# Hysocs/Aozora_SDXL_Training

Hardware: AMD Instinct MI355X
Metric: SDXL UNet train iters/sec (1024px, gbs=32) (higher is better)
Workload: dtype bf16; 1 GPU; SDXL-base UNet (2.567B params), epsilon pred, 1024x1024 (latent 4x128x128), ctx 77x2048, local batch 4 x grad-accum 8 x 1 GPU = global batch 32, Raven AdamW (bf16 m/v resident in HBM -- 10.3 GB of 288; the reference parks them in pinned host memory to fit 24 GB cards: other_configs.cfg2_state_on_host of --full --, sharded 1/N per rank), clip 1.0, eager 2-stream issue (dgrad chain || wgrad branch); global_batch=32, parallelism=dp1

## Files before the change

aozora_sdxl_training_amd/_lib.py:

```python
from __future__ import annotations

import ctypes
import os
import re
from typing import Callable, Dict, List, NamedTuple, Tuple

_HERE = os.path.dirname(os.path.abspath(__file__))
_ROOT = os.path.dirname(_HERE)
HEADER = os.path.join(_ROOT, "include", "aozora_hip.h")
LIB_PATH = os.path.join(_HERE, "libaozora_hip.so")

_CTYPES = {
    "int": ctypes.c_int, "long": ctypes.c_long, "float": ctypes.c_float,
    "void*": ctypes.c_void_p, "const void*": ctypes.c_void_p,
    "void**": ctypes.POINTER(ctypes.c_void_p), "int*": ctypes.POINTER(ctypes.c_int),
    "float*": ctypes.POINTER(ctypes.c_float), "const char*": ctypes.c_char_p, "long*": ctypes.POINTER(ctypes.c_long),
}


def parse_header(path: str = HEADER) -> Dict[str, Tuple[str, List[Tuple[str, str]]]]:
    src = open(path).read()
    src = re.sub(r"/\*.*?\*/", "", src, flags=re.S)
    protos = {}
    for m in re.finditer(r"\b(int|long)\s+(az_\w+)\s*\(([^)]*)\)\s*;", src):
        ret, name, args = m.group(1), m.group(2), m.group(3).strip()
        alist = []
        if args and args != "void":
            for a in args.split(","):
                a = " ".join(a.split())
                mm = re.match(r"(.*?)(\w+)$", a)
                ty = mm.group(1).strip().replace(" *", "*")
                alist.append((ty, mm.group(2)))
        protos[name] = (ret, alist)
    return protos


class AozoraError(RuntimeError):
    pass


class Call(NamedTuple):
    name: str
    args: tuple


class Record(NamedTuple):
    event: object
    stream: object


class Wait(NamedTuple):
    stream: object
    event: object


class Live(NamedTuple):
    fn: Callable
    args: tuple


class _Lib:
    def __init__(self):
        if not os.path.exists(LIB_PATH):
            raise AozoraError(
                f"{LIB_PATH} is missing: build it with `python -c 'import __graft_entry__ as g; g.build()'` "
                "(hipcc --offload-arch=gfx950). There is no CPU fallback for the HIP path.")
        self.cdll = ctypes.CDLL(LIB_PATH)
        self.protos = parse_header()
        self._fn = {}
        for name, (ret, args) in self.protos.items():
            fn = getattr(self.cdll, name)
            fn.restype = _CTYPES[ret]
            fn.argtypes = [_CTYPES[t] for t, _ in args]
            self._fn[name] = fn
        self.recorder = None

    def call(self, name: str, *args):
        fn = self._fn[name]
        rc = fn(*args)
        if rc != 0:
            raise AozoraError(f"{name} failed with code {rc}" + (" (argument error)" if rc <= -1000 else " (HIP error)"))
        if self.recorder is not None:
            self.recorder.append(Call(name, args))
        return rc

    def raw(self, name: str):
        return getattr(self.cdll, name)


def set_option(name: str, value: int):
    L = lib()
    rc = L._fn["az_set_option"](name.encode(), int(value))
    if rc != 0:
        raise AozoraError(f"az_set_option({name!r}) failed with code {rc}")


def get_option(name: str) -> int:
    v = ctypes.c_int()
    rc = lib()._fn["az_get_option"](name.encode(), ctypes.byref(v))
    if rc != 0:
        raise AozoraError(f"az_get_option({name!r}) failed with code {rc}")
    return v.value


class ForkEvent:
    __slots__ = ("cuda_event",)

    def __init__(self):
        h = ctypes.c_void_p()
        rc = lib()._fn["az_event_create_fork"](ctypes.byref(h))
        if rc != 0:
            raise AozoraError(f"az_event_create_fork failed with code {rc}")
        self.cuda_event = h.value

    def record(self, stream):
        rc = lib()._fn["az_event_record"](self.cuda_event, stream.cuda_stream)
        if rc != 0:
            raise AozoraError(f"az_event_record failed with code {rc}")

    def wait(self, stream):
        rc = lib()._fn["az_stream_wait_event"](stream.cuda_stream, self.cuda_event)
        if rc != 0:
            raise AozoraError(f"az_stream_wait_event failed with code {rc}")

    wait_on = wait

    def destroy(self):
        if self.cuda_event:
            lib()._fn["az_event_destroy"](self.cuda_event)
            self.cuda_event = None


_lib = None


def lib() -> _Lib:
    global _lib
    if _lib is None:
        _lib = _Lib()
    return _lib
```

aozora_sdxl_training_amd/csrc/az_common.h:

```cpp
#pragma once
#include <hip/hip_runtime.h>
#include <hip/hip_ext.h>
#include <stdint.h>
#include <tuple>
#include <utility>

typedef uint16_t bf16_t;
typedef __attribute__((ext_vector_type(8))) short bf16x8;
typedef __attribute__((ext_vector_type(4))) short bf16x4;
typedef __attribute__((ext_vector_type(4))) float f32x4;
typedef __attribute__((ext_vector_type(16))) float f32x16;
typedef __attribute__((ext_vector_type(4))) unsigned int u32x4;

#define AZ_OK 0
#define AZ_ERR_ARG(k) (-1000 - (k))

#define AZ_CHECK_LAUNCH()                          \
  do {                                             \
    hipError_t _e = hipGetLastError();             \
    if (_e != hipSuccess) return -(int)_e;         \
  } while (0)

hipEvent_t az_stop_event_of_this_thread();
template <typename... P, size_t... I>
// ... 25 lines not shown

__device__ __forceinline__ uint32_t pack2bf(float lo, float hi) {
  return (uint32_t)f2bf(lo) | ((uint32_t)f2bf(hi) << 16);
}

__device__ __forceinline__ float silu_f(float x) { return x * __builtin_amdgcn_rcpf(1.0f + __expf(-x)); }
__device__ __forceinline__ float dsilu_f(float x) {
  float s = __builtin_amdgcn_rcpf(1.0f + __expf(-x));
  return s * (1.0f + x * (1.0f - s));
}

__device__ __forceinline__ void gelu_pair(float g, float& gelu, float& dgelu) {
  const float x = fabsf(g) * 0.70710678118654752f;
  const float t = __builtin_amdgcn_rcpf(fmaf(0.3275911f, x, 1.0f));
  const float e = __expf(-x * x);
  const float poly = t * fmaf(t, fmaf(t, fmaf(t, fmaf(t, 1.061405429f, -1.453152027f), 1.421413741f), -0.284496736f), 0.254829592f);
  const float hc = 0.5f * poly * e;
  const float phi = g >= 0.f ? 1.0f - hc : hc;
  gelu = g * phi;
  dgelu = fmaf(g * 0.3989422804014327f, e, phi);
}
__device__ __forceinline__ float gelu_erf(float g) { float a, b; gelu_pair(g, a, b); return a; }
__device__ __forceinline__ float dgelu_erf(float g) { float a, b; gelu_pair(g, a, b); return b; }

__device__ __forceinline__ void divmod(long i, int d, long& q, int& r) {
  if ((unsigned long)i <= 0xFFFFFFFFul) {
    const unsigned qi = (unsigned)i / (unsigned)d;
    q = (long)qi; r = (int)((unsigned)i - qi * (unsigned)d);
  } else {
    q = i / d; r = (int)(i - q * d);
  }
}

__device__ __forceinline__ float wave_sum(float v) {
#pragma unroll
  for (int o = 32; o > 0; o >>= 1) v += __shfl_xor(v, o, 64);
  return v;
}
__device__ __forceinline__ float wave_max(float v) {
#pragma unroll
  for (int o = 32; o > 0; o >>= 1) v = fmaxf(v, __shfl_xor(v, o, 64));
  return v;
}

__device__ __forceinline__ float block_sum(float v, float* sh) {
  v = wave_sum(v);
  int w = threadIdx.x >> 6, nw = (blockDim.x + 63) >> 6;
  __syncthreads();
  if ((threadIdx.x & 63) == 0) sh[w] = v;
  __syncthreads();
  float r = 0.f;
  for (int i = 0; i < nw; ++i) r += sh[i];
  return r;
}

__device__ __forceinline__ bf16x4 lds_read_tr16_b64(uint32_t lds_byte_addr) {
  bf16x4 v;
  asm volatile("ds_read_b64_tr_b16 %0, %1" : "=v"(v) : "v"(lds_byte_addr) : "memory");
  return v;
}

enum AzOption {
  AZ_OPT_TILE_POLICY = 0,
  AZ_OPT_BIG_FILL,
  AZ_OPT_SPLIT_SLOTS,
  AZ_OPT_NOSPLIT_TILES,
  AZ_OPT_LDS_EXCLUSIVE,
  AZ_OPT_NT_SPLIT_BIG,
  AZ_OPT_NT_SPLIT_MINK,
  AZ_OPT_ATTN_SPLIT_TARGET,
  AZ_OPT_LN_RPB,
  AZ_OPT_INKERNEL_FINISH,
  AZ_OPT_NT_SPLIT2_MINK,
  AZ_OPT_GEMM_ABLATE,
  AZ_OPT_GEMM8,
  AZ_OPT_NT_SPLIT_FWD,
  AZ_OPT_ATTN_PIPE,
  AZ_OPT_XCD_SPLIT,
  AZ_OPT_ATTN_XCD,
  AZ_OPT_NORM_STAT_BF16,
  AZ_OPT_GN_RPT,
  AZ_OPT_GN_RPT_BWD,
  AZ_OPT_GN_RPT_APPLY,
  AZ_OPT_COUNT
};
int az_opt(int id);
```

aozora_sdxl_training_amd/csrc/az_gemm.hip:

```cpp
#include "az_common.h"
#include "aozora_hip.h"
#include <cstdlib>
#include <type_traits>

namespace {

constexpr int BK = 64;
constexpr int PITCH_K = BK * 2;
constexpr int PITCH_X = 128 * 2;

enum { A_ROW = 0, A_COL = 1, A_CONV = 2, A_CONVT = 3 };
enum { B_NT = 0, B_NN = 1, B_CONVDG = 2, B_CONVWG = 3 };

struct Geom {
  int Hin, Win, Cin;
  int Hout, Wout, Cout;
  int stride, pad, ks;
  int cpad;
  int ups;
};

struct Params {
  const bf16_t* A; const bf16_t* B;
  long lda, ldb;
// ... 1039 lines not shown
  if (g_force_bm == 256 && g_force_nw == 8) {
    p.bm = 256; p.bn = 256; p.nwaves = 0;
    return;
  }
  if (g_force_bm) {
    const bool kb32 = ((g_force_nw >> 5) & 1) && b_kmajor, deep = (g_force_nw >> 4) & 1;
    p.bm = g_force_bm; p.bn = g_force_bn; p.nwaves = g_force_nw & 15;
    p.kb = kb32 ? 32 : 64; p.stages = kb32 ? (deep ? 5 : 4) : (deep ? 3 : 2);
    if ((g_force_nw >> 6) & 1) { p.kb = 64; p.stages = 4; }
    if (p.bn == 160 && !b_kmajor) { p.bn = 128; p.nwaves = 8; p.stages = 2; }
    if (((g_force_nw >> 5) & 1) && !b_kmajor && p.bm == 256) { p.nwaves = 0; p.stages = 2; }
    return;
  }
  const int policy = az_opt(AZ_OPT_TILE_POLICY);
  const bool exclusive = az_opt(AZ_OPT_LDS_EXCLUSIVE) != 0;
  p.bm = 128; p.bn = 128; p.nwaves = 8;
  if (wgrad) return;
  const long t256 = (long)((p.M + 255) / 256) * ((p.N + 255) / 256);
  const long waves = (t256 + 255) / 256;
  const bool big = t256 * 10 >= waves * 256 * az_opt(AZ_OPT_BIG_FILL);
  if (b_kmajor && (p.N % 160) == 0 && (p.N <= 640 || !big)) {
    p.bn = 160; p.nwaves = 8;
    const long t160 = (long)((p.M + 127) / 128) * (p.N / 160);
    if ((policy >= 5 || exclusive) && t160 <= 256 && p.N > 640) p.stages = 3;
    return;
  }
  if (big) { p.bm = 256; p.bn = 256; p.nwaves = 0; }
}

int choose_split(Params& p, int want_split, long ws_bytes, bool wgrad = false, bool b_kmajor = false, bool big_split = false) {
  if (big_split) { p.bm = 256; p.bn = 256; p.nwaves = 0; p.stages = 2; p.kb = 64; }
  else choose_tile(p, wgrad, b_kmajor);
  p.tiles_m = (p.M + p.bm - 1) / p.bm;
  p.tiles_n = (p.N + p.bn - 1) / p.bn;
  const int ktiles = (p.K + BK - 1) / BK;
  int s = 1;
  if (want_split != 1 && p.ws) {
    const int tiles = p.tiles_m * p.tiles_n;
    if (want_split > 1) {
      s = want_split;
    } else {
      const int slots = az_opt(AZ_OPT_SPLIT_SLOTS);
      double best = -1.0;
      const int nosplit = az_opt(AZ_OPT_NOSPLIT_TILES);
      for (int c = 1; c <= (tiles >= nosplit ? 1 : 24); ++c) {
        if (c > 1 && ktiles / c < 8) break;
        const long blocks = (long)tiles * c;
        const double fill = (double)blocks / (double)(((blocks + slots - 1) / slots) * slots);
        const double score = fill / (1.0 + 0.08 * (c - 1));
        if (score > best + 1e-9) { best = score; s = c; }
      }
    }
    if (s > ktiles) s = ktiles;
    if (s > 64) s = 64;
    while (s > 1 && (long)s * p.M * p.N * 4 > ws_bytes) --s;
    if (s < 1) s = 1;
  }
  p.ktiles_per_split = (ktiles + s - 1) / s;
  p.ksplit = (ktiles + p.ktiles_per_split - 1) / p.ktiles_per_split;
  if (p.ksplit < 1) p.ksplit = 1;
  p.xsplit = (wgrad && az_opt(AZ_OPT_XCD_SPLIT) != 0 && p.ksplit > 1) ? 1 : 0;
  p.wgrad_c = wgrad ? 1 : 0;
  return AZ_OK;
}

void apply_gemm8(Params& p, int want_bn = 0) {
  p.use8 = 0;
  const bool forced = (g_force_bm == 256 && g_force_nw == 8);
  if (!forced && (g_force_bm || !az_opt(AZ_OPT_GEMM8))) return;
  if (p.bm != 256 || p.bn != 256 || (p.K % BK) || p.rowbias || !vec_epi_ok(p)) return;
  int bn = 256;
  if (forced) {
    bn = (g_force_bn == 320 && (p.N % 320) == 0) ? 320 : 256;
  } else if (want_bn) {
    bn = want_bn;
  } else if ((p.N % 320) == 0 && p.ksplit == 1) {
    auto fill = [&](int w) { const long tl = (long)((p.M + 255) / 256) * ((p.N + w - 1) / w); return (double)tl / (double)(((tl + 255) / 256) * 256); };
    if (fill(320) > fill(256) + 1e-9) bn = 320;
  }
  p.use8 = 1; p.bn = bn;
  p.tiles_m = (p.M + 255) / 256; p.tiles_n = (p.N + bn - 1) / bn;
}

}

extern "C" {

int az_gemm_set_exclusive(int on) { return az_set_option("LDS_EXCLUSIVE", on ? 1 : 0); }

int az_gemm_set_tile(int bm, int bn) { return az_gemm_set_tile_ex(bm, bn, 0); }

int az_gemm_set_tile_ex(int bm, int bn, int waves) {
  const bool std_tile = (bm == 128 && bn == 128 && (waves == 0 || waves == 8)) ||
                        (bm == 256 && bn == 256 && (waves == 0 || waves == 32 || waves == 8)) ||
                        (bm == 256 && bn == 320 && waves == 8);
  const bool n160 = (bm == 128 && bn == 160 && (waves == 0 || waves == 8 || waves == 24 ||
                                                waves == 40 || waves == 56 || waves == 72));
  if (!((bm == 0 && bn == 0) || std_tile || n160)) return AZ_ERR_ARG(9);
  g_force_bm = bm; g_force_bn = bn; g_force_nw = waves;
  return AZ_OK;
}

constexpr long TICKET_BYTES = 16384;
static void carve_tickets(Params& p, void* workspace, long& workspace_bytes) {
  p.tickets = nullptr;
  if (!workspace || workspace_bytes < TICKET_BYTES + 65536 || ((uintptr_t)workspace & 15) || (workspace_bytes & 15)) return;
  if (!az_opt(AZ_OPT_INKERNEL_FINISH)) return;
  workspace_bytes -= TICKET_BYTES;
  p.tickets = (unsigned*)((char*)workspace + workspace_bytes);
}

static int carve_colsum(Params& p, void* workspace, long& workspace_bytes, int nseg, int rps) {
  const long need = 64L * nseg * p.M * 4;
  if (!workspace || workspace_bytes < need + 4096 || ((uintptr_t)workspace & 15)) return AZ_ERR_ARG(20);
  if (nseg > 1 && (rps % BK)) return AZ_ERR_ARG(21);
  workspace_bytes = ((workspace_bytes - need) / 16) * 16;
  p.cs_ws = (float*)((char*)workspace + workspace_bytes);
  p.cs_nseg = nseg; p.cs_rps = rps;
  return AZ_OK;
}

static int gemm_impl(int transA, int transB, int M, int N, int K, const void* A, long lda, const void* B, long ldb,
                 void* C, long ldc, const void* bias, const void* rowbias, int rows_per_seg, long ld_rowbias,
                 const void* residual, long ldr, int accumulate, int split_k, void* workspace, long workspace_bytes,
                 void* bias_grad, int n_real, void* stream) {
  if (M <= 0 || N <= 0 || K <= 0) return AZ_ERR_ARG(1);
  if ((K & 7) && !transA && !transB) return AZ_ERR_ARG(2);
  if ((lda & 7) || (ldb & 7)) return AZ_ERR_ARG(3);
  if (((uintptr_t)A & 15) || ((uintptr_t)B & 15)) return AZ_ERR_ARG(4);
  if (rowbias && rows_per_seg <= 0) return AZ_ERR_ARG(5);
  Params p{};
  p.A = (const bf16_t*)A; p.B = (const bf16_t*)B; p.lda = lda; p.ldb = ldb; p.M = M; p.N = N; p.K = K;
  p.C = (bf16_t*)C; p.ldc = ldc; p.ws = (float*)workspace; p.bias = (const bf16_t*)bias;
  p.rowbias = (const bf16_t*)rowbias; p.rows_per_seg = rows_per_seg; p.ld_rb = ld_rowbias;
  p.R = (const bf16_t*)residual; p.ldr = ldr; p.accumulate = accumulate;
  carve_tickets(p, workspace, workspace_bytes);
  if (bias_grad) {
    if (!(transA && !transB) || n_real > M) return AZ_ERR_ARG(22);
    int rc0 = carve_colsum(p, workspace, workspace_bytes, 1, K);
    if (rc0) return rc0;
    p.cs_bias = (bf16_t*)bias_grad; p.cs_n_real = n_real; p.cs_seg_out = nullptr;
  }
  bool big_split = false; int split_bn = 256;
  {
    const int sb = az_opt(AZ_OPT_LDS_EXCLUSIVE) ? az_opt(AZ_OPT_NT_SPLIT_FWD) : az_opt(AZ_OPT_NT_SPLIT_BIG);
    if (sb > 1 && !transA && transB && !g_force_bm && !rowbias && workspace && (K % BK) == 0 && K >= az_opt(AZ_OPT_NT_SPLIT_MINK) &&
        (split_k == 0 || split_k == 1) && (!residual || (((ldr & 7) == 0) && (((uintptr_t)residual & 15) == 0))) &&
        ((N & 7) == 0) && ((ldc & 7) == 0) && (((uintptr_t)C & 15) == 0) && (((uintptr_t)workspace & 15) == 0)) {
      const int kt = K / BK;
      double best = 0.0; int bs = 0;
      for (int bn = 256; bn <= 320; bn += 64) {
        if (bn == 320 && ((N % 320) || !az_opt(AZ_OPT_GEMM8))) continue;
        const long tl = (long)((M + 255) / 256) * ((N + bn - 1) / bn);
        if (tl > 128) continue;
        for (int sp = 2; sp <= sb; ++sp) {
          if (kt / sp < 8 || tl * sp > 256 || (long)sp * M * N * 4 > workspace_bytes) break;
          const double score = (double)(tl * sp) / 256.0 - 0.02 * (sp - 1);
          if (score > best + 1e-9) { best = score; bs = sp; split_bn = bn; }
        }
      }
      if (bs > 1 && best >= 0.7) { big_split = true; split_k = bs; }
    }
  }
  if (!big_split && !transA && transB && !g_force_bm && !rowbias && !residual && workspace && (K % BK) == 0 && (split_k == 0 || split_k == 1) &&
      !az_opt(AZ_OPT_LDS_EXCLUSIVE) && az_opt(AZ_OPT_TILE_POLICY) < 5) {
    const int mink = az_opt(AZ_OPT_NT_SPLIT2_MINK);
    const long t256 = (long)((M + 255) / 256) * ((N + 255) / 256);
    const long t160 = (long)((M + 127) / 128) * (N / 160);
    const bool big = t256 * 10 >= ((t256 + 255) / 256) * 256 * az_opt(AZ_OPT_BIG_FILL);
    if (mink > 0 && K >= mink && (N % 160) == 0 && N > 640 && !big && t160 <= 256 && 2L * M * N * 4 <= workspace_bytes - 65536) split_k = 2;
  }
  choose_split(p, split_k, workspace_bytes, transA != 0, !transA && transB, big_split);
  if (p.ksplit > 1 && (rowbias || (residual && !vec_epi_ok(p)))) return AZ_ERR_ARG(6);
  if (!transA && transB) apply_gemm8(p, big_split ? split_bn : 0);
  if ((long)p.tiles_m * p.tiles_n > TICKET_BYTES / 4 || (long)p.ksplit * p.M * p.N * 4 >= 0x7FFFFFF0L || p.use8 || (p.R && p.ksplit > 1)) p.tickets = nullptr;
  hipStream_t st = (hipStream_t)stream;
  if (p.tickets) AZ_HIP(hipMemsetAsync(p.tickets, 0, (size_t)p.tiles_m * p.tiles_n * 4, st));
  int rc;
  if (!transA && transB) rc = launch<A_ROW, B_NT>(p, st);
  else if (!transA && !transB) rc = launch<A_ROW, B_NN>(p, st);
  else if (transA && !transB) rc = launch<A_COL, B_NN>(p, st);
  else return AZ_ERR_ARG(7);
  if (rc) return rc;
  return finish_product(p, st, nullptr, bias_grad, n_real);
}

int az_gemm_bf16(int transA, int transB, int M, int N, int K, const void* A, long lda, const void* B, long ldb,
                 void* C, long ldc, const void* bias, const void* rowbias, int rows_per_seg, long ld_rowbias,
                 const void* residual, long ldr, int accumulate, int split_k, void* workspace, long workspace_bytes,
                 void* stream) {
  return gemm_impl(transA, transB, M, N, K, A, lda, B, ldb, C, ldc, bias, rowbias, rows_per_seg, ld_rowbias, residual, ldr,
                   accumulate, split_k, workspace, workspace_bytes, nullptr, 0, stream);
}

int az_gemm_geglu_fwd_bf16(int M, int H, int K, const void* X, long lda, const void* W, long ldb, const void* bias, void* proj, long ldp,
                           void* out, long ldo, void* stream) {
  if (M <= 0 || H <= 0 || K <= 0 || (K & 7) || (H & 7)) return AZ_ERR_ARG(72);
  if ((lda & 7) || (ldb & 7) || (ldp & 7) || (ldo & 7)) return AZ_ERR_ARG(73);
  if (((uintptr_t)X & 15) || ((uintptr_t)W & 15) || ((uintptr_t)proj & 15) || ((uintptr_t)out & 15) || !proj || !out) return AZ_ERR_ARG(74);
  Params p{};
  p.A = (const bf16_t*)X; p.B = (const bf16_t*)W; p.lda = lda; p.ldb = ldb; p.M = M; p.N = 2 * H; p.K = K;
  p.C = (bf16_t*)proj; p.ldc = ldp; p.bias = (const bf16_t*)bias; p.gg_H = H; p.gg_y = (bf16_t*)out; p.gg_ldy = ldo;
  choose_split(p, 1, 0, false, true);
  const bool big = (p.bm == 256 && p.bn == 256);
  p.stages = 2; p.kb = 64;
  if (!big) { p.bm = 128; p.bn = 128; }
  p.nwaves = big ? 0 : 8;
  p.tiles_m = (M + p.bm - 1) / p.bm; p.tiles_n = (H + p.bn / 2 - 1) / (p.bn / 2);
  p.use8 = (big && (K % BK) == 0 && vec_epi_ok(p) && (az_opt(AZ_OPT_GEMM8) || (g_force_bm == 256 && g_force_nw == 8)) &&
            (!g_force_bm || g_force_nw == 8)) ? 1 : 0;
  return launch<A_ROW, B_NT>(p, (hipStream_t)stream);
}

int az_gemm_nt_grouped_bf16(int M, int K, const void* A, long lda, const void* groups_dev, int ngroups, long total_tiles_n, void* stream) {
  if (M <= 0 || K <= 0 || (K & 7) || (lda & 7) || ((uintptr_t)A & 15) || !groups_dev || ngroups <= 0 || total_tiles_n <= 0 ||
      ((uintptr_t)groups_dev & 7)) return AZ_ERR_ARG(70);
  Params p{};
  p.A = (const bf16_t*)A; p.lda = lda; p.M = M; p.K = K; p.N = 0;
  p.groups = (const GemmGroup*)groups_dev; p.ngroups = ngroups;
  p.bm = 128; p.bn = 160; p.nwaves = 8; p.kb = 64;
  p.stages = az_opt(AZ_OPT_LDS_EXCLUSIVE) ? 3 : 2;
  p.tiles_m = (M + 127) / 128;
  if ((long)p.tiles_m * total_tiles_n > 0x7FFFFFF0L) return AZ_ERR_ARG(71);
  p.tiles_n = (int)total_tiles_n;
  p.ksplit = 1; p.ktiles_per_split = (K + BK - 1) / BK;
  if ((long)M * lda * 2 >= 0x7FFFFFF0L) return AZ_ERR_ARG(8);
  p.lda2 = (int)(lda * 2);
  p.k_full = (K % BK) == 0;
  p.vec_epi = 1;
  hipStream_t st = (hipStream_t)stream;
  if (p.stages == 3) return launch_tile<A_ROW, B_NT, 128, 160, 4, 2, 3, 64, 1>(p, st);
  return launch_tile<A_ROW, B_NT, 128, 160, 4, 2, 2, 64, 1>(p, st);
}

int az_gemm_tn_grouped_bf16(const void* groups_dev, int ngroups, long total_tiles, void* stream) {
  if (!groups_dev || ngroups <= 0 || total_tiles <= 0 || total_tiles > 0x7FFFFFF0L || ((uintptr_t)groups_dev & 7)) return AZ_ERR_ARG(75);
  Params p{};
  p.tgroups = (const TnGroup*)groups_dev; p.ngroups = ngroups;
  p.bm = 128; p.bn = 128; p.nwaves = 8; p.kb = 64; p.stages = 2;
  p.tiles_m = (int)total_tiles; p.tiles_n = 1;
  p.ksplit = 1; p.accumulate = 1;
  return launch_tile<A_COL, B_NN, 128, 128, 4, 2, 2, 64, 3>(p, (hipStream_t)stream);
}

int az_gemm_wgrad_bias_bf16(int M, int N, int K, const void* dY, long lddy, const void* X, long ldx, void* dW, long lddw,
                            int accumulate, int split_k, void* workspace, long workspace_bytes, void* bias_grad, int n_real,
                            void* stream) {
  if (!bias_grad) return AZ_ERR_ARG(22);
  return gemm_impl(1, 0, M, N, K, dY, lddy, X, ldx, dW, lddw, nullptr, nullptr, 0, 0, nullptr, 0, accumulate, split_k, workspace,
                   workspace_bytes, bias_grad, n_real, stream);
}

static int conv_impl(int mode, int batch, int Hin, int Win, int Cin, int Hout, int Wout, int Cout, int ksize, int stride,
                   int pad, int cpad, const void* X, long ldx, const void* W, const void* dY, long lddy, void* out,
                   long ldo, const void* bias, const void* rowbias, long ld_rowbias, const void* residual, long ldr,
                   int accumulate, int split_k, void* workspace, long workspace_bytes, void* bias_grad, void* seg_grad,
                   void* stream) {
  const int ups = (mode >> 4) & 1;
  mode &= 15;
  if (ups && ((mode != 0 && mode != 2) || ksize != 3 || stride != 1 || (Hin & 1) || (Win & 1))) return AZ_ERR_ARG(23);
  if (ksize != 1 && ksize != 3) return AZ_ERR_ARG(10);
  if (stride != 1 && stride != 2) return AZ_ERR_ARG(11);
  if ((Cin & 7)) return AZ_ERR_ARG(12);
  Params p{};
  p.g = Geom{Hin, Win, Cin, Hout, Wout, Cout, stride, pad, ksize, cpad > 0 ? cpad : Cout, ups};
  const int taps = ksize * ksize;
  p.bias = (const bf16_t*)bias; p.accumulate = accumulate; p.ws = (float*)workspace;
  p.rowbias = (const bf16_t*)rowbias; p.ld_rb = ld_rowbias; p.R = (const bf16_t*)residual; p.ldr = ldr;
  hipStream_t st = (hipStream_t)stream;
  int rc;
  if (mode == 0) {
    p.A = (const bf16_t*)X; p.lda = ldx; p.B = (const bf16_t*)W; p.ldb = (long)taps * Cin;
    p.M = batch * Hout * Wout; p.N = Cout; p.K = taps * Cin; p.C = (bf16_t*)out; p.ldc = ldo;
    p.rows_per_seg = Hout * Wout;
    p.tap_uniform = (Cin % BK) == 0;
// ... 70 lines not shown
```

aozora_sdxl_training_amd/csrc/az_norm.hip:

```cpp
#include "az_common.h"
#include "aozora_hip.h"

namespace {

constexpr int GN_MAX_THREADS = 256;

struct GnGeom {
  int B, HW, C, G, cpg, cchunks, py, rows_per_chunk, nchunk;
  int stat_bf16;
};

__device__ __forceinline__ float stat_round(float v, int on) { return on ? bf2f(f2bf(v)) : v; }

constexpr int GN_RPT_MIN = 4;
__host__ GnGeom gn_geom(int B, int HW, int C, int G, int pass = -1) {
  GnGeom g;
  g.B = B; g.HW = HW; g.C = C; g.G = G; g.cpg = C / G; g.cchunks = C / 8;
  g.py = GN_MAX_THREADS / g.cchunks; if (g.py < 1) g.py = 1;
  int want = (HW + 1023) / 1024;
  int rpt = pass < 0 ? GN_RPT_MIN : az_opt(pass == 2 ? AZ_OPT_GN_RPT_APPLY : pass ? AZ_OPT_GN_RPT_BWD : AZ_OPT_GN_RPT);
  if (rpt < GN_RPT_MIN) rpt = GN_RPT_MIN; if (rpt > 64) rpt = 64;
  if (want < rpt * g.py) want = rpt * g.py;
  g.rows_per_chunk = ((want + g.py - 1) / g.py) * g.py;
  g.nchunk = (HW + g.rows_per_chunk - 1) / g.rows_per_chunk;
// ... 287 lines not shown
      ub[i] = *reinterpret_cast<const uint4*>(beta + cc * 8);
      unpack8(ux, v[i]);
#pragma unroll
      for (int e = 0; e < 8; ++e) s += v[i][e];
    }
  }
  const float invC = 1.0f / (float)C;
  const float mean = wave_sum(s) * invC;
  float q = 0.f;
#pragma unroll
  for (int i = 0; i < LN_MAXCH; ++i) {
    int cc = lane + 64 * i;
    if (cc < cch) {
#pragma unroll
      for (int e = 0; e < 8; ++e) { float d = v[i][e] - mean; q += d * d; }
    }
  }
  const float rstd = rsqrtf(fmaf(wave_sum(q), invC, eps));
  if (lane == 0) { stats[row * 2] = stat_round(mean, stat_bf16); stats[row * 2 + 1] = stat_round(rstd, stat_bf16); }
#pragma unroll
  for (int i = 0; i < LN_MAXCH; ++i) {
    int cc = lane + 64 * i;
    if (cc < cch) {
      float g8[8], b8[8], o[8];
      unpack8(ug[i], g8);
      unpack8(ub[i], b8);
#pragma unroll
      for (int e = 0; e < 8; ++e) o[e] = (v[i][e] - mean) * rstd * g8[e] + b8[e];
      *reinterpret_cast<uint4*>(y + (long)row * ldy + cc * 8) = pack8(o);
    }
  }
}

template <int NCH>
__global__ __launch_bounds__(256) void ln_bwd_dx_kernel(int M, int C, const bf16_t* __restrict__ x, long ldx, const bf16_t* __restrict__ gamma,
                                 const float* __restrict__ stats, const bf16_t* __restrict__ dy, long lddy,
                                 bf16_t* dx, long lddx, const bf16_t* dadd, long ldadd) {
  const bool accumulate = dadd != nullptr;
  const int lane = threadIdx.x & 63;
  const int row = blockIdx.x * (blockDim.x >> 6) + (threadIdx.x >> 6);
  if (row >= M) return;
  const int cch = C >> 3;
  const float mean = stats[row * 2], rstd = stats[row * 2 + 1];
  float xh[NCH][8], dg[NCH][8];
  uint4 prev[NCH];
  float c1 = 0.f, c2 = 0.f;
#pragma unroll
  for (int i = 0; i < NCH; ++i) {
    const int cc = lane + 64 * i;
    if (cc < cch) {
      const uint4 ux = *reinterpret_cast<const uint4*>(x + (long)row * ldx + cc * 8);
      const uint4 ud = *reinterpret_cast<const uint4*>(dy + (long)row * lddy + cc * 8);
      const uint4 ug = *reinterpret_cast<const uint4*>(gamma + cc * 8);
      if (accumulate) prev[i] = *reinterpret_cast<const uint4*>(dadd + (long)row * ldadd + cc * 8);
      float f[8], d[8], g8[8];
      unpack8(ux, f); unpack8(ud, d); unpack8(ug, g8);
#pragma unroll
      for (int e = 0; e < 8; ++e) {
        xh[i][e] = (f[e] - mean) * rstd;
        dg[i][e] = d[e] * g8[e];
        c1 += dg[i][e]; c2 += dg[i][e] * xh[i][e];
      }
    }
  }
  const float invC = 1.0f / (float)C;
  c1 = wave_sum(c1) * invC; c2 = wave_sum(c2) * invC;
#pragma unroll
  for (int i = 0; i < NCH; ++i) {
    const int cc = lane + 64 * i;
    if (cc < cch) {
      float o[8];
      bf16_t* op = dx + (long)row * lddx + cc * 8;
      if (accumulate) unpack8(prev[i], o);
#pragma unroll
      for (int e = 0; e < 8; ++e) {
        float vv = rstd * (dg[i][e] - c1 - xh[i][e] * c2);
        o[e] = accumulate ? o[e] + vv : vv;
      }
      *reinterpret_cast<uint4*>(op) = pack8(o);
    }
  }
}

template <int NCH>
__global__ __launch_bounds__(256) void ln_bwd_fused_kernel(int M, int C, int rows_per_block, const bf16_t* __restrict__ x, long ldx,
                                 const bf16_t* __restrict__ gamma, const float* __restrict__ stats, const bf16_t* __restrict__ dy,
                                 long lddy, bf16_t* dx, long lddx, const bf16_t* dadd, long ldadd, float* __restrict__ partial) {
  const bool accumulate = dadd != nullptr;
  extern __shared__ float sh[];
  const int lane = threadIdx.x & 63, w = threadIdx.x >> 6;
  const int cch = C >> 3;
  const int r0 = blockIdx.x * rows_per_block;
  int r1 = r0 + rows_per_block; if (r1 > M) r1 = M;
  float pg[NCH][8], pb[NCH][8];
  uint4 ug[NCH];
#pragma unroll
  for (int i = 0; i < NCH; ++i) {
    const int cc = lane + 64 * i;
    ug[i] = cc < cch ? *reinterpret_cast<const uint4*>(gamma + cc * 8) : make_uint4(0, 0, 0, 0);
#pragma unroll
    for (int e = 0; e < 8; ++e) { pg[i][e] = 0.f; pb[i][e] = 0.f; }
  }
  const float invC = 1.0f / (float)C;
  uint4 nx[NCH], nd[NCH], np[NCH];
  float nmean = 0.f, nrstd = 0.f;
  auto fetch = [&](int row) {
    nmean = stats[row * 2]; nrstd = stats[row * 2 + 1];
#pragma unroll
    for (int i = 0; i < NCH; ++i) {
      const int cc = lane + 64 * i;
      if (cc < cch) {
        nx[i] = *reinterpret_cast<const uint4*>(x + (long)row * ldx + cc * 8);
        nd[i] = *reinterpret_cast<const uint4*>(dy + (long)row * lddy + cc * 8);
        if (accumulate) np[i] = *reinterpret_cast<const uint4*>(dadd + (long)row * ldadd + cc * 8);
      }
    }
  };
  if (r0 + w < r1) fetch(r0 + w);
  for (int row = r0 + w; row < r1; row += 4) {
    const float mean = nmean, rstd = nrstd;
    uint4 cx[NCH], cd[NCH], prev[NCH];
#pragma unroll
    for (int i = 0; i < NCH; ++i) { cx[i] = nx[i]; cd[i] = nd[i]; if (accumulate) prev[i] = np[i]; }
    if (row + 4 < r1) fetch(row + 4);
    float xh[NCH][8], dg[NCH][8];
    float c1 = 0.f, c2 = 0.f;
#pragma unroll
    for (int i = 0; i < NCH; ++i) {
      const int cc = lane + 64 * i;
      if (cc < cch) {
        float f[8], d[8], g8[8];
        unpack8(cx[i], f); unpack8(cd[i], d); unpack8(ug[i], g8);
#pragma unroll
        for (int e = 0; e < 8; ++e) {
          xh[i][e] = (f[e] - mean) * rstd;
          pb[i][e] += d[e]; pg[i][e] += d[e] * xh[i][e];
          dg[i][e] = d[e] * g8[e];
          c1 += dg[i][e]; c2 += dg[i][e] * xh[i][e];
        }
      }
    }
    c1 = wave_sum(c1) * invC; c2 = wave_sum(c2) * invC;
#pragma unroll
    for (int i = 0; i < NCH; ++i) {
      const int cc = lane + 64 * i;
      if (cc < cch) {
        float o[8];
        if (accumulate) unpack8(prev[i], o);
#pragma unroll
        for (int e = 0; e < 8; ++e) {
          float vv = rstd * (dg[i][e] - c1 - xh[i][e] * c2);
          o[e] = accumulate ? o[e] + vv : vv;
        }
        *reinterpret_cast<uint4*>(dx + (long)row * lddx + cc * 8) = pack8(o);
      }
    }
  }
  float* out = partial + (long)blockIdx.x * C * 2;
#pragma unroll
  for (int i = 0; i < NCH; ++i) {
    if (i) __syncthreads();
    float* d = sh + ((long)w * 64 + lane) * 16;
#pragma unroll
    for (int e = 0; e < 8; e += 2)
      *reinterpret_cast<float4*>(d + e * 2) = make_float4(pg[i][e], pb[i][e], pg[i][e + 1], pb[i][e + 1]);
    __syncthreads();
    const int l2 = threadIdx.x >> 2, q = threadIdx.x & 3;
    const int cc = l2 + 64 * i;
    if (cc < cch) {
      float4 a = *reinterpret_cast<const float4*>(sh + (long)l2 * 16 + q * 4);
#pragma unroll
      for (int y = 1; y < 4; ++y) {
        const float4 v = *reinterpret_cast<const float4*>(sh + ((long)y * 64 + l2) * 16 + q * 4);
        a.x += v.x; a.y += v.y; a.z += v.z; a.w += v.w;
      }
      *reinterpret_cast<float4*>(out + ((long)cc * 8 + q * 2) * 2) = a;
    }
  }
}

__global__ void ln_bwd_param_kernel(int M, int C, int rows_per_block, const bf16_t* __restrict__ x, long ldx,
                                    const float* __restrict__ stats, const bf16_t* __restrict__ dy, long lddy,
                                    float* __restrict__ partial) {
  extern __shared__ float sh[];
  const int cc = blockIdx.y * blockDim.x + threadIdx.x;
  const int cch = C >> 3;
  const int r0 = blockIdx.x * rows_per_block;
  int r1 = r0 + rows_per_block; if (r1 > M) r1 = M;
  float dg[8], db[8];
#pragma unroll
  for (int e = 0; e < 8; ++e) { dg[e] = 0.f; db[e] = 0.f; }
  if (cc < cch) {
#pragma unroll 4
    for (int r = r0 + threadIdx.y; r < r1; r += blockDim.y) {
      const float mean = stats[r * 2], rstd = stats[r * 2 + 1];
      float f[8], d[8];
      unpack8(*reinterpret_cast<const uint4*>(x + (long)r * ldx + cc * 8), f);
      unpack8(*reinterpret_cast<const uint4*>(dy + (long)r * lddy + cc * 8), d);
#pragma unroll
      for (int e = 0; e < 8; ++e) { db[e] += d[e]; dg[e] += d[e] * (f[e] - mean) * rstd; }
    }
  }
  const int w8 = blockDim.x * 8;
#pragma unroll
  for (int e = 0; e < 8; ++e) {
    sh[((threadIdx.y * w8) + threadIdx.x * 8 + e) * 2] = dg[e];
    sh[((threadIdx.y * w8) + threadIdx.x * 8 + e) * 2 + 1] = db[e];
  }
  __syncthreads();
  const int tid = threadIdx.y * blockDim.x + threadIdx.x, nth = blockDim.x * blockDim.y;
  for (int lc = tid; lc < w8; lc += nth) {
    const int c = blockIdx.y * w8 + lc;
    if (c >= C) continue;
    float a = 0.f, bsum = 0.f;
    for (int y = 0; y < (int)blockDim.y; ++y) { a += sh[(y * w8 + lc) * 2]; bsum += sh[(y * w8 + lc) * 2 + 1]; }
    partial[((long)blockIdx.x * C + c) * 2] = a;
    partial[((long)blockIdx.x * C + c) * 2 + 1] = bsum;
  }
}

__device__ __forceinline__ void colpair_finalize_block(int blk, int nparts, int C, const float* __restrict__ partial, bf16_t* dgamma, bf16_t* dbeta,
                                                       float4 (*sh)[16]) {
  const int lc = threadIdx.x & 15, sl = threadIdx.x >> 4;
  const int c = blk * 32 + lc * 2;
  float4 a = make_float4(0.f, 0.f, 0.f, 0.f);
  if (c < C) {
    const float* base = partial + (long)c * 2;
    int k = sl;
    for (; k + 7 * 16 < nparts; k += 8 * 16) {
      float4 v[8];
#pragma unroll
      for (int u = 0; u < 8; ++u) v[u] = *reinterpret_cast<const float4*>(base + (long)(k + u * 16) * C * 2);
#pragma unroll
      for (int u = 0; u < 8; ++u) { a.x += v[u].x; a.y += v[u].y; a.z += v[u].z; a.w += v[u].w; }
    }
    for (; k < nparts; k += 16) {
      const float4 v = *reinterpret_cast<const float4*>(base + (long)k * C * 2);
      a.x += v.x; a.y += v.y; a.z += v.z; a.w += v.w;
    }
  }
  sh[sl][lc] = a;
  __syncthreads();
  if (sl == 0 && c < C) {
    a = make_float4(0.f, 0.f, 0.f, 0.f);
#pragma unroll
    for (int i = 0; i < 16; ++i) { const float4 v = sh[i][lc]; a.x += v.x; a.y += v.y; a.z += v.z; a.w += v.w; }
    if (dgamma) { dgamma[c] = f2bf(bf2f(dgamma[c]) + a.x); dgamma[c + 1] = f2bf(bf2f(dgamma[c + 1]) + a.z); }
    if (dbeta) { dbeta[c] = f2bf(bf2f(dbeta[c]) + a.y); dbeta[c + 1] = f2bf(bf2f(dbeta[c + 1]) + a.w); }
  }
}
// ... 57 lines not shown
                       (const bf16_t*)beta, (const float*)stats, (bf16_t*)y, ldy);
  AZ_CHECK_LAUNCH();
  return AZ_OK;
}

int az_groupnorm_bwd_ex(int batch, int HW, int C, int G, int fuse_silu, const void* x, long ldx, const void* gamma,
                        const void* beta, const void* stats, const void* dy, long lddy, void* dx, long lddx,
                        const void* dx_add, long ld_add, void* dgamma, void* dbeta, void* partial, void* stream) {
  int rc = gn_check(batch, HW, C, G, ldx); if (rc) return rc;
  if ((lddy & 7) || (lddx & 7) || (dx_add && (ld_add & 7)) || ((uintptr_t)gamma & 15) || ((uintptr_t)beta & 15) || ((uintptr_t)stats & 7)) return AZ_ERR_ARG(25);
  GnGeom g = gn_geom(batch, HW, C, G, 1);
  hipStream_t st = (hipStream_t)stream;
  dim3 blk(g.cchunks, g.py), grid(g.nchunk, batch);
  size_t shb = (size_t)g.py * C * 2 * sizeof(float);
  if (shb > 64 * 1024) return AZ_ERR_ARG(24);
  float* part = (float*)partial;
  float* chan = part + (long)batch * g.nchunk * C * 2;
  float* gsum = chan + (long)batch * C * 2;
  if (fuse_silu)
    az_launch(gn_bwd_partial_kernel<true>, grid, blk, shb, st, g, (const bf16_t*)x, ldx, (const bf16_t*)gamma,
                       (const bf16_t*)beta, (const float*)stats, (const bf16_t*)dy, lddy, part);
  else
    az_launch(gn_bwd_partial_kernel<false>, grid, blk, shb, st, g, (const bf16_t*)x, ldx, (const bf16_t*)gamma,
                       (const bf16_t*)beta, (const float*)stats, (const bf16_t*)dy, lddy, part);
  AZ_CHECK_LAUNCH();
  az_launch(gn_bwd_finalize_kernel, dim3(G, batch), dim3(64, 16), 0, st, g, (const bf16_t*)gamma, (const float*)part, chan, gsum);
  AZ_CHECK_LAUNCH();
  const bool params = dgamma || dbeta;
  if (params && !dx) {
    az_launch(gn_bwd_param_kernel, dim3((C + 255) / 256), dim3(256), 0, st, g, (const float*)chan, (bf16_t*)dgamma, (bf16_t*)dbeta);
    AZ_CHECK_LAUNCH();
  }
  const float* chan_for_apply = params ? chan : nullptr;
  if (dx) {
    g = gn_geom(batch, HW, C, G, 2);
    blk = dim3(g.cchunks, g.py); grid = dim3(g.nchunk, batch);
    if (fuse_silu)
      az_launch(gn_bwd_apply_kernel<true>, grid, blk, 0, st, g, (const bf16_t*)x, ldx, (const bf16_t*)gamma,
                         (const bf16_t*)beta, (const float*)stats, (const float*)gsum, (const bf16_t*)dy, lddy,
                         (bf16_t*)dx, lddx, (const bf16_t*)dx_add, ld_add, chan_for_apply, (bf16_t*)dgamma, (bf16_t*)dbeta);
    else
      az_launch(gn_bwd_apply_kernel<false>, grid, blk, 0, st, g, (const bf16_t*)x, ldx, (const bf16_t*)gamma,
                         (const bf16_t*)beta, (const float*)stats, (const float*)gsum, (const bf16_t*)dy, lddy,
                         (bf16_t*)dx, lddx, (const bf16_t*)dx_add, ld_add, chan_for_apply, (bf16_t*)dgamma, (bf16_t*)dbeta);
    AZ_CHECK_LAUNCH();
  }
  return AZ_OK;
}

int az_groupnorm_bwd(int batch, int HW, int C, int G, int fuse_silu, const void* x, long ldx, const void* gamma,
                     const void* beta, const void* stats, const void* dy, long lddy, void* dx, long lddx,
                     int accumulate_dx, void* dgamma, void* dbeta, void* partial, void* stream) {
  return az_groupnorm_bwd_ex(batch, HW, C, G, fuse_silu, x, ldx, gamma, beta, stats, dy, lddy, dx, lddx, accumulate_dx ? dx : nullptr, lddx,
                             dgamma, dbeta, partial, stream);
}

long az_ln_scratch_floats(int M, int C) { (void)M; return (long)LN_FUSED_MAX_BLOCKS * C * 2; }

int az_layernorm_fwd(int M, int C, float eps, const void* x, long ldx, const void* gamma, const void* beta, void* y,
                     long ldy, void* stats, void* stream) {
  if (M <= 0 || (C & 7) || C > 64 * 8 * LN_MAXCH || (ldx & 7) || (ldy & 7)) return AZ_ERR_ARG(30);
  az_launch(ln_fwd_kernel, dim3((M + 3) / 4), dim3(256), 0, (hipStream_t)stream, M, C, eps, (const bf16_t*)x, ldx,
                     (const bf16_t*)gamma, (const bf16_t*)beta, (bf16_t*)y, ldy, (float*)stats, (int)(az_opt(AZ_OPT_NORM_STAT_BF16) != 0));
  AZ_CHECK_LAUNCH();
  return AZ_OK;
}

static int ln_fused_rpb(int M);
int az_layernorm_bwd_ex(int M, int C, const void* x, long ldx, const void* gamma, const void* stats, const void* dy,
                        long lddy, void* dx, long lddx, const void* dx_add, long ld_add, void* dgamma, void* dbeta, void* partial,
                        void* stream) {
  if (M <= 0 || (C & 7) || C > 64 * 8 * LN_MAXCH || (ldx & 7) || (lddy & 7) || (dx && (lddx & 7)) || (dx_add && (ld_add & 7))) return AZ_ERR_ARG(31);
  hipStream_t st = (hipStream_t)stream;
  const int cch = C / 8;
  const int nch = (cch + 63) / 64;
  dim3 g1((M + 3) / 4), b1(256);
#define LN_DX(N) az_launch(ln_bwd_dx_kernel<N>, g1, b1, 0, st, M, C, (const bf16_t*)x, ldx, (const bf16_t*)gamma, \
                                    (const float*)stats, (const bf16_t*)dy, lddy, (bf16_t*)dx, lddx, (const bf16_t*)dx_add, ld_add)
  if (dx && (dgamma || dbeta)) {
    const int nblk = (M + ln_fused_rpb(M) - 1) / ln_fused_rpb(M);
    const int rpb = ((M + nblk - 1) / nblk + 3) / 4 * 4;
    const size_t shb = (size_t)4 * 64 * 16 * sizeof(float);
#define LN_FU(N) az_launch(ln_bwd_fused_kernel<N>, dim3(nblk), b1, shb, st, M, C, rpb, (const bf16_t*)x, ldx, (const bf16_t*)gamma, \
                                    (const float*)stats, (const bf16_t*)dy, lddy, (bf16_t*)dx, lddx, (const bf16_t*)dx_add, ld_add, (float*)partial)
    if (nch == 1) LN_FU(1); else if (nch == 2) LN_FU(2); else if (nch == 3) LN_FU(3); else LN_FU(4);
#undef LN_FU
    AZ_CHECK_LAUNCH();
    az_launch(colpair_finalize_kernel, dim3((C + 31) / 32), dim3(256), 0, st, nblk, C, (const float*)partial,
                       (bf16_t*)dgamma, (bf16_t*)dbeta);
    AZ_CHECK_LAUNCH();
    return AZ_OK;
  }
  if (dx) {
    if (nch == 1) LN_DX(1); else if (nch == 2) LN_DX(2); else if (nch == 3) LN_DX(3); else LN_DX(4);
    AZ_CHECK_LAUNCH();
  }
#undef LN_DX
  if (dgamma || dbeta) {
    int bx = cch < 128 ? cch : 128; int by = 256 / bx; if (by < 1) by = 1; if (by > 16) by = 16;
    int colblocks = (cch + bx - 1) / bx;
    int rpb = (M + LN_BWD_BLOCKS - 1) / LN_BWD_BLOCKS; if (rpb < by) rpb = by;
    int nblk = (M + rpb - 1) / rpb;
    size_t shb = (size_t)by * bx * 8 * 2 * sizeof(float);
    az_launch(ln_bwd_param_kernel, dim3(nblk, colblocks), dim3(bx, by), shb, st, M, C, rpb, (const bf16_t*)x, ldx,
                       (const float*)stats, (const bf16_t*)dy, lddy, (float*)partial);
    AZ_CHECK_LAUNCH();
    az_launch(colpair_finalize_kernel, dim3((C + 31) / 32), dim3(256), 0, st, nblk, C, (const float*)partial,
                       (bf16_t*)dgamma, (bf16_t*)dbeta);
    AZ_CHECK_LAUNCH();
  }
  return AZ_OK;
}

static int ln_fused_rpb(int M) {
  const int rpb_env = az_opt(AZ_OPT_LN_RPB);
  int rpb = rpb_env < 4 ? 4 : (rpb_env + 3) / 4 * 4;
  while ((M + rpb - 1) / rpb > LN_FUSED_MAX_BLOCKS) rpb += 4;
  return rpb;
}

int az_ln_partial_blocks(int M) { return M > 0 ? (M + ln_fused_rpb(M) - 1) / ln_fused_rpb(M) : 0; }

int az_layernorm_bwd_partial(int M, int C, const void* x, long ldx, const void* gamma, const void* stats, const void* dy,
                             long lddy, void* dx, long lddx, const void* dx_add, long ld_add, void* partial, int nblk, void* stream) {
  if (M <= 0 || (C & 7) || C > 64 * 8 * LN_MAXCH || (ldx & 7) || (lddy & 7) || !dx || (lddx & 7) || (dx_add && (ld_add & 7)) || !partial) return AZ_ERR_ARG(32);
  if (nblk <= 0 || nblk > LN_FUSED_MAX_BLOCKS) return AZ_ERR_ARG(34);
  const int rpb = ((M + nblk - 1) / nblk + 3) / 4 * 4;
  if ((M + rpb - 1) / rpb != nblk) return AZ_ERR_ARG(34);
  hipStream_t st = (hipStream_t)stream;
  const int nch = (C / 8 + 63) / 64;
  const size_t shb = (size_t)4 * 64 * 16 * sizeof(float);
#define LN_FU(N) az_launch(ln_bwd_fused_kernel<N>, dim3(nblk), dim3(256), shb, st, M, C, rpb, (const bf16_t*)x, ldx, (const bf16_t*)gamma, \
                                    (const float*)stats, (const bf16_t*)dy, lddy, (bf16_t*)dx, lddx, (const bf16_t*)dx_add, ld_add, (float*)partial)
  if (nch == 1) LN_FU(1); else if (nch == 2) LN_FU(2); else if (nch == 3) LN_FU(3); else LN_FU(4);
#undef LN_FU
  AZ_CHECK_LAUNCH();
  return AZ_OK;
}

int az_ln_param_finish_multi(const void* jobs_dev, int njobs, long nblocks, void* stream) {
  if (!jobs_dev || njobs <= 0 || nblocks <= 0 || nblocks > 0x7FFFFFF0L || ((uintptr_t)jobs_dev & 7)) return AZ_ERR_ARG(33);
  az_launch(colpair_finalize_multi_kernel, dim3((unsigned)nblocks), dim3(256), 0, (hipStream_t)stream, (const LnFinishJob*)jobs_dev, njobs);
  AZ_CHECK_LAUNCH();
  return AZ_OK;
}

int az_layernorm_bwd(int M, int C, const void* x, long ldx, const void* gamma, const void* stats, const void* dy,
                     long lddy, void* dx, long lddx, int accumulate_dx, void* dgamma, void* dbeta, void* partial,
                     void* stream) {
  return az_layernorm_bwd_ex(M, C, x, ldx, gamma, stats, dy, lddy, dx, lddx, accumulate_dx ? dx : nullptr, lddx, dgamma, dbeta, partial, stream);
}

}
```

aozora_sdxl_training_amd/csrc/az_runtime.hip:

```cpp
#include "az_common.h"
#include "aozora_hip.h"
#include <string.h>
#include <stdlib.h>
#include <atomic>
#include <mutex>

namespace {
struct OptDef { const char* name; int def; };
const OptDef OPT_DEFS[AZ_OPT_COUNT] = {
  {"TILE_POLICY", 4}, {"BIG_FILL", 5}, {"SPLIT_SLOTS", 384}, {"NOSPLIT_TILES", 256}, {"LDS_EXCLUSIVE", 0}, {"NT_SPLIT_BIG", 3},
  {"NT_SPLIT_MINK", 5120}, {"ATTN_SPLIT_TARGET", 384}, {"LN_RPB", 32}, {"INKERNEL_FINISH", 0}, {"NT_SPLIT2_MINK", 0}, {"GEMM_ABLATE", 0}, {"GEMM8", 1}, {"NT_SPLIT_FWD", 0}, {"ATTN_PIPE", 15}, {"XCD_SPLIT", 1}, {"ATTN_XCD", 15}, {"NORM_STAT_BF16", 1}, {"GN_RPT", 4}, {"GN_RPT_BWD", 32}, {"GN_RPT_APPLY", 32},
};
std::atomic<int> g_opt[AZ_OPT_COUNT];
std::once_flag g_opt_once;
void opt_init() {
  for (int i = 0; i < AZ_OPT_COUNT; ++i) {
    char key[64];
    snprintf(key, sizeof key, "AZ_%s", OPT_DEFS[i].name);
    const char* e = getenv(key);
    g_opt[i].store(e ? atoi(e) : OPT_DEFS[i].def, std::memory_order_relaxed);
  }
}

__global__ void spin_kernel(long ticks) {
  const long t0 = (long)wall_clock64();
  while ((long)wall_clock64() - t0 < ticks) __builtin_amdgcn_s_sleep(32);
}
}

struct AzContext { int device; std::atomic<int> refs; std::atomic<int> opt[AZ_OPT_COUNT]; };
static void ctx_release(AzContext* c) {
  if (c && c->refs.fetch_sub(1, std::memory_order_acq_rel) == 1) delete c;
}
struct AzCurrent {
  AzContext* c = nullptr;
  ~AzCurrent() { ctx_release(c); }
  operator AzContext*() const { return c; }
  AzContext* operator->() const { return c; }
  void set(AzContext* n) {
    if (n == c) return;
    if (n) n->refs.fetch_add(1, std::memory_order_relaxed);
    AzContext* old = c; c = n;
    ctx_release(old);
  }
};
static thread_local AzCurrent t_ctx;

int az_opt(int id) {
  std::call_once(g_opt_once, opt_init);
  AzContext* c = t_ctx.c;
  return c ? c->opt[id].load(std::memory_order_relaxed) : g_opt[id].load(std::memory_order_relaxed);
}

struct AzStopEvent { hipEvent_t ev = nullptr; long launches = 0; };
static AzStopEvent& az_stop_event_slot() {
  static thread_local AzStopEvent s;
  return s;
}
hipEvent_t az_stop_event_of_this_thread() {
  AzStopEvent& s = az_stop_event_slot();
  if (s.ev) ++s.launches;
  return s.ev;
}

extern "C" {

int az_version(void) { return 101; }

int az_set_option(const char* name, int value) {
  std::call_once(g_opt_once, opt_init);
  if (!name) return AZ_ERR_ARG(91);
  std::atomic<int>* tab = t_ctx.c ? t_ctx.c->opt : g_opt;
  for (int i = 0; i < AZ_OPT_COUNT; ++i)
    if (!strcmp(name, OPT_DEFS[i].name)) { tab[i].store(value, std::memory_order_relaxed); return AZ_OK; }
  return AZ_ERR_ARG(92);
}

int az_get_option(const char* name, int* value) {
  std::call_once(g_opt_once, opt_init);
  if (!name || !value) return AZ_ERR_ARG(91);
  std::atomic<int>* tab = t_ctx.c ? t_ctx.c->opt : g_opt;
  for (int i = 0; i < AZ_OPT_COUNT; ++i)
    if (!strcmp(name, OPT_DEFS[i].name)) { *value = tab[i].load(std::memory_order_relaxed); return AZ_OK; }
  return AZ_ERR_ARG(92);
}

int az_init(int device, void** handle) {
  std::call_once(g_opt_once, opt_init);
  if (!handle || device < 0) return AZ_ERR_ARG(93);
  AzContext* c = new AzContext;
  c->device = device;
  c->refs.store(1, std::memory_order_relaxed);
  for (int i = 0; i < AZ_OPT_COUNT; ++i) c->opt[i].store(g_opt[i].load(std::memory_order_relaxed), std::memory_order_relaxed);
  *handle = c;
// ... 111 lines not shown
```

aozora_sdxl_training_amd/csrc/az_tape_dispatch.inc:

```
static const char* const AZ_TAPE_FN_NAMES[] = {
  "az_adamw8bit_step",
  "az_adamw_flat",
  "az_adamw_flat_ex",
  "az_add_rows",
  "az_attn_bwd",
  "az_attn_fwd",
  "az_clip_coef",
  "az_colsum",
  "az_colsum_grad",
  "az_conv2d_bf16",
  "az_conv2d_wgrad_bias_bf16",
  "az_destroy",
  "az_event_destroy",
  "az_event_record",
  "az_event_sync",
  "az_f32_to_bf16",
  "az_geglu_bwd",
  "az_geglu_fwd",
  "az_gemm_bf16",
  "az_gemm_geglu_fwd_bf16",
  "az_gemm_nt_grouped_bf16",
  "az_gemm_set_exclusive",
  "az_gemm_set_tile",
  "az_gemm_set_tile_ex",
  "az_gemm_tn_grouped_bf16",
  "az_gemm_wgrad_bias_bf16",
  "az_graph_begin",
  "az_graph_destroy",
  "az_graph_launch",
  "az_groupnorm_bwd",
  "az_groupnorm_bwd_ex",
  "az_groupnorm_fwd",
  "az_host_free",
  "az_layernorm_bwd",
  "az_layernorm_bwd_ex",
  "az_layernorm_bwd_partial",
  "az_layernorm_fwd",
  "az_ln_param_finish_multi",
  "az_ln_partial_blocks",
  "az_make_current",
  "az_memcpy_async",
  "az_memset_async",
  "az_mse_loss_fwd_bwd",
  "az_nchw_to_nhwc_pad",
  "az_nhwc_to_nchw",
  "az_noise_target",
  "az_raven_step",
  "az_raven_step_ex",
  "az_reduce_segs_to_bf16",
  "az_scale_bf16",
  "az_scale_f32",
  "az_set_launch_stop_event",
  "az_silu_bwd",
  "az_silu_fwd",
  "az_spin",
  "az_stage_inputs",
  "az_stream_sync",
  "az_stream_wait_event",
  "az_sumsq",
  "az_sumsq_bf16",
  "az_timestep_embed",
  "az_titan_offload",
  "az_transpose_bf16",
  "az_transpose_bf16_batched",
  "az_transpose_multi_bf16",
  "az_upsample2x_bwd",
  "az_upsample2x_fwd",
  "az_version",
};
static const int AZ_TAPE_FN_NARGS[] = {7, 9, 10, 9, 35, 19, 6, 8, 10, 29, 22, 1, 1, 2, 1, 4, 9, 7, 22, 13, 8, 1, 2, 3, 4, 16, 1, 1, 2, 19, 20, 15, 1, 15, 16, 15, 11, 4, 1, 1, 5, 4, 14, 8, 8, 12, 13, 14, 6, 4, 4, 1, 6, 4, 2, 8, 1, 2, 7, 6, 6, 6, 7, 10, 4, 7, 7, 0};
static int az_tape_dispatch(int fn, const long* w) {
  switch (fn) {
    case 0: return az_adamw8bit_step((int)w[0], (const void*)w[1], (long)w[2], (const void*)w[3], (const void*)w[4], (const void*)w[5], (void*)w[6]);
    case 1: return az_adamw_flat((long)w[0], (void*)w[1], (const void*)w[2], (void*)w[3], (void*)w[4], (int)w[5], (const void*)w[6], (const void*)w[7], (void*)w[8]);
    case 2: return az_adamw_flat_ex((long)w[0], (void*)w[1], (const void*)w[2], (int)w[3], (void*)w[4], (void*)w[5], (int)w[6], (const void*)w[7], (const void*)w[8], (void*)w[9]);
    case 3: return az_add_rows((long)w[0], (int)w[1], (const void*)w[2], (long)w[3], (const void*)w[4], (long)w[5], (void*)w[6], (long)w[7], (void*)w[8]);
    case 4: return az_attn_bwd((int)w[0], (int)w[1], (int)w[2], (int)w[3], word_float(w[4]), (const void*)w[5], (long)w[6], (long)w[7], (const void*)w[8], (long)w[9], (long)w[10], (const void*)w[11], (long)w[12], (long)w[13], (const void*)w[14], (long)w[15], (long)w[16], (const void*)w[17], (long)w[18], (long)w[19], (const void*)w[20], (void*)w[21], (void*)w[22], (long)w[23], (long)w[24], (void*)w[25], (long)w[26], (long)w[27], (void*)w[28], (long)w[29], (long)w[30], (void*)w[31], (long)w[32], (int)w[33], (void*)w[34]);
    case 5: return az_attn_fwd((int)w[0], (int)w[1], (int)w[2], (int)w[3], word_float(w[4]), (const void*)w[5], (long)w[6], (long)w[7], (const void*)w[8], (long)w[9], (long)w[10], (const void*)w[11], (long)w[12], (long)w[13], (void*)w[14], (long)w[15], (long)w[16], (void*)w[17], (void*)w[18]);
    case 6: return az_clip_coef((const void*)w[0], word_float(w[1]), word_float(w[2]), (void*)w[3], (void*)w[4], (void*)w[5]);
    case 7: return az_colsum((long)w[0], (int)w[1], (int)w[2], (const void*)w[3], (long)w[4], (void*)w[5], (void*)w[6], (void*)w[7]);
    case 8: return az_colsum_grad((long)w[0], (int)w[1], (int)w[2], (const void*)w[3], (long)w[4], (void*)w[5], (void*)w[6], (int)w[7], (void*)w[8], (void*)w[9]);
    case 9: return az_conv2d_bf16((int)w[0], (int)w[1], (int)w[2], (int)w[3], (int)w[4], (int)w[5], (int)w[6], (int)w[7], (int)w[8], (int)w[9], (int)w[10], (int)w[11], (const void*)w[12], (long)w[13], (const void*)w[14], (const void*)w[15], (long)w[16], (void*)w[17], (long)w[18], (const void*)w[19], (const void*)w[20], (long)w[21], (const void*)w[22], (long)w[23], (int)w[24], (int)w[25], (void*)w[26], (long)w[27], (void*)w[28]);
    case 10: return az_conv2d_wgrad_bias_bf16((int)w[0], (int)w[1], (int)w[2], (int)w[3], (int)w[4], (int)w[5], (int)w[6], (int)w[7], (int)w[8], (int)w[9], (const void*)w[10], (long)w[11], (const void*)w[12], (long)w[13], (void*)w[14], (int)w[15], (int)w[16], (void*)w[17], (long)w[18], (void*)w[19], (void*)w[20], (void*)w[21]);
    case 11: return az_destroy((void*)w[0]);
    case 12: return az_event_destroy((void*)w[0]);
    case 13: return az_event_record((void*)w[0], (void*)w[1]);
    case 14: return az_event_sync((void*)w[0]);
    case 15: return az_f32_to_bf16((long)w[0], (const void*)w[1], (void*)w[2], (void*)w[3]);
    case 16: return az_geglu_bwd((int)w[0], (int)w[1], (const void*)w[2], (long)w[3], (const void*)w[4], (long)w[5], (void*)w[6], (long)w[7], (void*)w[8]);
    case 17: return az_geglu_fwd((int)w[0], (int)w[1], (const void*)w[2], (long)w[3], (void*)w[4], (long)w[5], (void*)w[6]);
    case 18: return az_gemm_bf16((int)w[0], (int)w[1], (int)w[2], (int)w[3], (int)w[4], (const void*)w[5], (long)w[6], (const void*)w[7], (long)w[8], (void*)w[9], (long)w[10], (const void*)w[11], (const void*)w[12], (int)w[13], (long)w[14], (const void*)w[15], (long)w[16], (int)w[17], (int)w[18], (void*)w[19], (long)w[20], (void*)w[21]);
    case 19: return az_gemm_geglu_fwd_bf16((int)w[0], (int)w[1], (int)w[2], (const void*)w[3], (long)w[4], (const void*)w[5], (long)w[6], (const void*)w[7], (void*)w[8], (long)w[9], (void*)w[10], (long)w[11], (void*)w[12]);
    case 20: return az_gemm_nt_grouped_bf16((int)w[0], (int)w[1], (const void*)w[2], (long)w[3], (const void*)w[4], (int)w[5], (long)w[6], (void*)w[7]);
    case 21: return az_gemm_set_exclusive((int)w[0]);
    case 22: return az_gemm_set_tile((int)w[0], (int)w[1]);
    case 23: return az_gemm_set_tile_ex((int)w[0], (int)w[1], (int)w[2]);
    case 24: return az_gemm_tn_grouped_bf16((const void*)w[0], (int)w[1], (long)w[2], (void*)w[3]);
    case 25: return az_gemm_wgrad_bias_bf16((int)w[0], (int)w[1], (int)w[2], (const void*)w[3], (long)w[4], (const void*)w[5], (long)w[6], (void*)w[7], (long)w[8], (int)w[9], (int)w[10], (void*)w[11], (long)w[12], (void*)w[13], (int)w[14], (void*)w[15]);
    case 26: return az_graph_begin((void*)w[0]);
    case 27: return az_graph_destroy((void*)w[0]);
    case 28: return az_graph_launch((void*)w[0], (void*)w[1]);
    case 29: return az_groupnorm_bwd((int)w[0], (int)w[1], (int)w[2], (int)w[3], (int)w[4], (const void*)w[5], (long)w[6], (const void*)w[7], (const void*)w[8], (const void*)w[9], (const void*)w[10], (long)w[11], (void*)w[12], (long)w[13], (int)w[14], (void*)w[15], (void*)w[16], (void*)w[17], (void*)w[18]);
    case 30: return az_groupnorm_bwd_ex((int)w[0], (int)w[1], (int)w[2], (int)w[3], (int)w[4], (const void*)w[5], (long)w[6], (const void*)w[7], (const void*)w[8], (const void*)w[9], (const void*)w[10], (long)w[11], (void*)w[12], (long)w[13], (const void*)w[14], (long)w[15], (void*)w[16], (void*)w[17], (void*)w[18], (void*)w[19]);
    case 31: return az_groupnorm_fwd((int)w[0], (int)w[1], (int)w[2], (int)w[3], word_float(w[4]), (int)w[5], (const void*)w[6], (long)w[7], (const void*)w[8], (const void*)w[9], (void*)w[10], (long)w[11], (void*)w[12], (void*)w[13], (void*)w[14]);
    case 32: return az_host_free((void*)w[0]);
    case 33: return az_layernorm_bwd((int)w[0], (int)w[1], (const void*)w[2], (long)w[3], (const void*)w[4], (const void*)w[5], (const void*)w[6], (long)w[7], (void*)w[8], (long)w[9], (int)w[10], (void*)w[11], (void*)w[12], (void*)w[13], (void*)w[14]);
    case 34: return az_layernorm_bwd_ex((int)w[0], (int)w[1], (const void*)w[2], (long)w[3], (const void*)w[4], (const void*)w[5], (const void*)w[6], (long)w[7], (void*)w[8], (long)w[9], (const void*)w[10], (long)w[11], (void*)w[12], (void*)w[13], (void*)w[14], (void*)w[15]);
    case 35: return az_layernorm_bwd_partial((int)w[0], (int)w[1], (const void*)w[2], (long)w[3], (const void*)w[4], (const void*)w[5], (const void*)w[6], (long)w[7], (void*)w[8], (long)w[9], (const void*)w[10], (long)w[11], (void*)w[12], (int)w[13], (void*)w[14]);
    case 36: return az_layernorm_fwd((int)w[0], (int)w[1], word_float(w[2]), (const void*)w[3], (long)w[4], (const void*)w[5], (const void*)w[6], (void*)w[7], (long)w[8], (void*)w[9], (void*)w[10]);
    case 37: return az_ln_param_finish_multi((const void*)w[0], (int)w[1], (long)w[2], (void*)w[3]);
    case 38: return az_ln_partial_blocks((int)w[0]);
    case 39: return az_make_current((void*)w[0]);
    case 40: return az_memcpy_async((void*)w[0], (const void*)w[1], (long)w[2], (int)w[3], (void*)w[4]);
    case 41: return az_memset_async((void*)w[0], (int)w[1], (long)w[2], (void*)w[3]);
    case 42: return az_mse_loss_fwd_bwd((int)w[0], (int)w[1], (int)w[2], (const void*)w[3], (long)w[4], (const void*)w[5], (const void*)w[6], word_float(w[7]), (void*)w[8], (void*)w[9], (void*)w[10], (int)w[11], (void*)w[12], (void*)w[13]);
    case 43: return az_nchw_to_nhwc_pad((int)w[0], (int)w[1], (int)w[2], (int)w[3], (const void*)w[4], (int)w[5], (void*)w[6], (void*)w[7]);
    case 44: return az_nhwc_to_nchw((int)w[0], (int)w[1], (int)w[2], (int)w[3], (const void*)w[4], (void*)w[5], (int)w[6], (void*)w[7]);
    case 45: return az_noise_target((int)w[0], (int)w[1], (int)w[2], (int)w[3], (int)w[4], (const void*)w[5], (const void*)w[6], (const void*)w[7], (const void*)w[8], (void*)w[9], (void*)w[10], (void*)w[11]);
    case 46: return az_raven_step((long)w[0], (void*)w[1], (const void*)w[2], (void*)w[3], (void*)w[4], (int)w[5], (const void*)w[6], (const void*)w[7], (void*)w[8], (long)w[9], (void*)w[10], (void*)w[11], (void*)w[12]);
    case 47: return az_raven_step_ex((long)w[0], (void*)w[1], (const void*)w[2], (int)w[3], (void*)w[4], (void*)w[5], (int)w[6], (const void*)w[7], (const void*)w[8], (void*)w[9], (long)w[10], (void*)w[11], (void*)w[12], (void*)w[13]);
    case 48: return az_reduce_segs_to_bf16((int)w[0], (int)w[1], (const void*)w[2], (void*)w[3], (int)w[4], (void*)w[5]);
    case 49: return az_scale_bf16((long)w[0], (void*)w[1], (const void*)w[2], (void*)w[3]);
    case 50: return az_scale_f32((long)w[0], (void*)w[1], (const void*)w[2], (void*)w[3]);
    case 51: return az_set_launch_stop_event((void*)w[0]);
    case 52: return az_silu_bwd((long)w[0], (const void*)w[1], (const void*)w[2], (void*)w[3], (int)w[4], (void*)w[5]);
    case 53: return az_silu_fwd((long)w[0], (const void*)w[1], (void*)w[2], (void*)w[3]);
    case 54: return az_spin((long)w[0], (void*)w[1]);
    case 55: return az_stage_inputs((int)w[0], (const void*)w[1], (const void*)w[2], (const void*)w[3], (int)w[4], (const void*)w[5], (void*)w[6], (void*)w[7]);
    case 56: return az_stream_sync((void*)w[0]);
    case 57: return az_stream_wait_event((void*)w[0], (void*)w[1]);
    case 58: return az_sumsq((long)w[0], (const void*)w[1], (int)w[2], (void*)w[3], (int)w[4], (void*)w[5], (void*)w[6]);
    case 59: return az_sumsq_bf16((long)w[0], (const void*)w[1], (void*)w[2], (int)w[3], (void*)w[4], (void*)w[5]);
    case 60: return az_timestep_embed((int)w[0], (int)w[1], (const void*)w[2], (void*)w[3], (long)w[4], (void*)w[5]);
    case 61: return az_titan_offload((long)w[0], (const void*)w[1], (void*)w[2], (void*)w[3], (int)w[4], (void*)w[5]);
    case 62: return az_transpose_bf16((int)w[0], (int)w[1], (const void*)w[2], (long)w[3], (void*)w[4], (long)w[5], (void*)w[6]);
    case 63: return az_transpose_bf16_batched((int)w[0], (int)w[1], (int)w[2], (const void*)w[3], (long)w[4], (long)w[5], (void*)w[6], (long)w[7], (long)w[8], (void*)w[9]);
    case 64: return az_transpose_multi_bf16((const void*)w[0], (int)w[1], (long)w[2], (void*)w[3]);
    case 65: return az_upsample2x_bwd((int)w[0], (int)w[1], (int)w[2], (int)w[3], (const void*)w[4], (void*)w[5], (void*)w[6]);
    case 66: return az_upsample2x_fwd((int)w[0], (int)w[1], (int)w[2], (int)w[3], (const void*)w[4], (void*)w[5], (void*)w[6]);
    case 67: return az_version();
    default: return AZ_ERR_ARG(60);
  }
}
```

aozora_sdxl_training_amd/ops.py:

```python
from __future__ import annotations

import ctypes
from typing import Optional

import torch

from ._lib import lib, AozoraError

BF16 = torch.bfloat16
F32 = torch.float32


def _ptr(t: Optional[torch.Tensor]):
    return ctypes.c_void_p(t.data_ptr()) if t is not None else ctypes.c_void_p(0)


def _stream():
    return ctypes.c_void_p(torch.cuda.current_stream().cuda_stream)


def _req(cond, msg):
    if not cond:
        raise AozoraError("operand check failed: " + msg)

# ... 41 lines not shown
        return self

    def __exit__(self, *a):
        if PROFILER is not None:
            lib().call("az_event_record", self.e1, _stream())
            PROFILER.add(self.key, self.flops, self.nbytes, self.e0, self.e1)
        return False


class Workspace:

    def __init__(self, device, splitk_bytes: int = 192 << 20, scratch_floats: int = 64 << 20, attn_bytes: int = 96 << 20):
        self.device = device
        self.splitk = torch.zeros(splitk_bytes // 4, dtype=F32, device=device)
        self.attn = torch.empty(attn_bytes // 4, dtype=F32, device=device)
        self.scratch = torch.empty(scratch_floats, dtype=F32, device=device)
        self.small = torch.zeros(4096 + 64, dtype=F32, device=device)


_ws = {}


_ws_slot = [0]


def set_workspace_slot(slot: int):
    _ws_slot[0] = slot


def workspace(device=None) -> Workspace:
    device = torch.device(device if device is not None else f"cuda:{torch.cuda.current_device()}")
    if device.index is None:
        device = torch.device("cuda", torch.cuda.current_device())
    key = (device, _ws_slot[0])
    if key not in _ws:
        _ws[key] = Workspace(device)
    return _ws[key]



def gemm(a, b, out, *, trans_a=False, trans_b=True, bias=None, rowbias=None, rows_per_seg=0, residual=None,
         accumulate=False, split_k=1, bias_grad=None):
    ar, ac, lda = _rows(a)
    br, bc, ldb = _rows(b)
    M, K = (ac, ar) if trans_a else (ar, ac)
    N, Kb = (br, bc) if trans_b else (bc, br)
    _req(K == Kb, f"K mismatch {K} vs {Kb}")
    _req(not (trans_a and trans_b), "transA & transB unsupported")
    om, on, ldc = _rows(out)
    _req((om, on) == (M, N), f"out shape {(om, on)} != {(M, N)}")
    _req(lda % 8 == 0 and ldb % 8 == 0, "lda/ldb must be multiples of 8")
    _req(a.data_ptr() % 16 == 0 and b.data_ptr() % 16 == 0, "A/B must be 16-byte aligned")
    if not trans_a and trans_b:
        _req(K % 8 == 0, "K must be a multiple of 8")
    if trans_a:
        _req(a.shape[1] % 8 == 0 or lda >= ((M + 7) // 8) * 8, "transposed A rows must be readable in 8-element chunks")
    if not trans_b:
        _req(ldb >= ((N + 7) // 8) * 8, "B rows must be readable in 8-element chunks")
    if bias is not None:
        _req(bias.dtype == BF16 and bias.numel() == N and bias.is_contiguous(), "bias must be contiguous bf16 [N]")
    ld_rb = 0
    if rowbias is not None:
        rr, rc, ld_rb = _rows(rowbias)
        _req(rc == N and rows_per_seg > 0 and rr * rows_per_seg >= M, "rowbias shape")
    ldr = 0
    if residual is not None:
        rm, rn, ldr = _rows(residual)
        _req((rm, rn) == (M, N), "residual shape")
    ws = workspace(out.device)
    if bias_grad is not None:
        _req(trans_a and not trans_b and bias is None and rowbias is None and residual is None, "bias_grad needs the wgrad form")
        _req(bias_grad.dtype == BF16 and bias_grad.is_contiguous() and bias_grad.numel() <= M, "bias_grad must be contiguous bf16 [<=M]")
        with _prof("gemm_tn" + (f" {M}x{N}x{K}+b" if PROFILE_SHAPES else ""), 2.0 * M * N * K, 2.0 * (M * K + N * K + M * N)):
            lib().call("az_gemm_wgrad_bias_bf16", M, N, K, _ptr(a), lda, _ptr(b), ldb, _ptr(out), ldc, int(accumulate), int(split_k),
                       _ptr(ws.splitk), ws.splitk.numel() * 4, _ptr(bias_grad), bias_grad.numel(), _stream())
        return out
    with _prof("gemm_" + ("tn" if trans_a else ("nt" if trans_b else "nn")) + (f" {M}x{N}x{K}" if PROFILE_SHAPES else ""), 2.0 * M * N * K, 2.0 * (M * K + N * K + M * N)):
      lib().call("az_gemm_bf16", int(trans_a), int(trans_b), M, N, K, _ptr(a), lda, _ptr(b), ldb, _ptr(out), ldc,
               _ptr(bias), _ptr(rowbias), int(rows_per_seg), ld_rb, _ptr(residual), ldr, int(accumulate), int(split_k),
               _ptr(ws.splitk), ws.splitk.numel() * 4, _stream())
    return out


def gemm_nt_grouped(a, table, ngroups: int, total_tiles_n: int, sum_n: int = 0):
    M, K, lda = _rows(a)
    _req(K % 8 == 0 and lda % 8 == 0 and a.data_ptr() % 16 == 0, "grouped gemm: A layout")
    with _prof("gemm_nt" + (f" grouped {M}x{sum_n}x{K} ({ngroups})" if PROFILE_SHAPES else ""), 2.0 * M * sum_n * K,
               2.0 * (M * K + sum_n * K + M * sum_n)):
        lib().call("az_gemm_nt_grouped_bf16", M, K, _ptr(a), lda, _ptr(table), int(ngroups), int(total_tiles_n), _stream())


def tn_group_table(jobs, device):
    recs, tiles, flops, nbytes = [], 0, 0.0, 0.0
    for dy, x, dw, bg in sorted(jobs, key=lambda j: -j[0].shape[0]):
        K, M, lda = _rows(dy)
        Kx, N, ldb = _rows(x)
        Mw, Nw, ldc = _rows(dw)
        _req(Kx == K and (Mw, Nw) == (M, N), f"grouped wgrad shapes {tuple(dy.shape)} {tuple(x.shape)} {tuple(dw.shape)}")
        _req(lda % 8 == 0 and ldb % 8 == 0 and dy.data_ptr() % 16 == 0 and x.data_ptr() % 16 == 0, "grouped wgrad: operand alignment")
        _req((M % 8 == 0 or lda >= ((M + 7) // 8) * 8) and ldb >= ((N + 7) // 8) * 8, "grouped wgrad: rows must be readable in 8-element chunks")
        _req((K * lda + M + 8) * 2 < 0x7FFFFFF0 and (K * ldb + N + 8) * 2 < 0x7FFFFFF0, "grouped wgrad: operand extent >= 2 GiB")
        n_real = 0
        if bg is not None:
            _req(bg.dtype == BF16 and bg.is_contiguous() and bg.numel() <= M, "grouped wgrad: bias_grad must be contiguous bf16 [<= M]")
            n_real = bg.numel()
        vec = int(N % 8 == 0 and ldc % 8 == 0 and dw.data_ptr() % 16 == 0)
        tm, tn = (M + 127) // 128, (N + 127) // 128
        recs.append([dy.data_ptr(), x.data_ptr(), dw.data_ptr(), bg.data_ptr() if bg is not None else 0, M, N, K, lda, ldb, ldc, tiles, tm, tn, n_real, vec, 0])
        tiles += tm * tn
        flops += 2.0 * M * N * K
        nbytes += 2.0 * (M * K + N * K + M * N)
    return torch.tensor(recs, dtype=torch.int64, device=device), len(recs), tiles, flops, nbytes


def gemm_tn_grouped(table, ngroups: int, total_tiles: int, flops: float = 0.0, nbytes: float = 0.0):
    with _prof("gemm_tn" + (f" grouped ({ngroups}) {total_tiles} tiles" if PROFILE_SHAPES else ""), flops, nbytes):
        lib().call("az_gemm_tn_grouped_bf16", _ptr(table), int(ngroups), int(total_tiles), _stream())


def gemm_geglu_fwd(x, w, bias, proj, out):
    M, K, lda = _rows(x)
    H2, Kw, ldb = _rows(w)
    Mp, H2p, ldp = _rows(proj)
    Mo, H, ldo = _rows(out)
    _req(Kw == K and H2 == 2 * H and (Mp, Mo, H2p) == (M, M, H2) and (bias is None or bias.numel() == H2), "fused GEGLU forward shapes")
    with _prof("gemm_nt" + (f" {M}x{H2}x{K}+geglu" if PROFILE_SHAPES else ""), 2.0 * M * H2 * K, 2.0 * (M * K + H2 * K + M * H2 + M * H)):
        lib().call("az_gemm_geglu_fwd_bf16", M, H, K, _ptr(x), lda, _ptr(w), ldb, _ptr(bias), _ptr(proj), ldp, _ptr(out), ldo, _stream())
    return out


def _nhwc(t: torch.Tensor):
    _req(t.is_cuda and t.dtype == BF16 and t.dim() == 4, "need cuda bf16 (B,H,W,C)")
    B, H, W, C = t.shape
    ld = t.stride(2)
    _req(t.stride(3) == 1 and t.stride(1) == W * ld and t.stride(0) == H * W * ld, f"non-uniform NHWC strides {t.stride()}")
    _req(ld % 8 == 0 and t.data_ptr() % 16 == 0, "pixel stride must be a multiple of 8 and base 16-byte aligned")
    return B, H, W, C, ld


def conv_fwd(x, w, out, *, stride=1, bias=None, rowbias=None, residual=None, upsample=False):
    B, H, W, Cin, ldx = _nhwc(x)
    if upsample:
        _req(stride == 1 and w.shape[1] == 3, "the upsample gather exists for 3x3 stride-1 convolutions")
        H, W = 2 * H, 2 * W
    _req(w.dtype == BF16 and w.is_contiguous() and w.dim() == 4 and w.shape[3] == Cin and w.shape[1] == w.shape[2], "weight layout")
    Cout, ks = w.shape[0], w.shape[1]
    pad = 1 if ks == 3 else 0
    Ho = (H + 2 * pad - ks) // stride + 1
    Wo = (W + 2 * pad - ks) // stride + 1
    _req(out.is_cuda and out.dtype == BF16 and tuple(out.shape) == (B, Ho, Wo, Cout) and out.stride(3) == 1, "out shape")
    ldo = out.stride(2)
    _req(out.stride(1) == Wo * ldo and out.stride(0) == Ho * Wo * ldo, "out strides")
    ld_rb = 0
    if rowbias is not None:
        _req(rowbias.dtype == BF16 and tuple(rowbias.shape) == (B, Cout) and rowbias.stride(1) == 1, "rowbias [B][Cout]")
        ld_rb = rowbias.stride(0)
    ldr = 0
    if residual is not None:
        _req(tuple(residual.shape) == tuple(out.shape) and residual.stride(3) == 1, "residual shape")
        ldr = residual.stride(2)
    if bias is not None:
        _req(bias.dtype == BF16 and bias.numel() == Cout and bias.is_contiguous(), "bias")
    with _prof('conv_fwd' + (f' {B}x{H}x{W} {Cin}->{Cout} k{ks}s{stride}' if PROFILE_SHAPES else ''), 2.0 * B * Ho * Wo * Cout * ks * ks * Cin, 0.0):
        lib().call("az_conv2d_bf16", 16 if upsample else 0, B, H, W, Cin, Ho, Wo, Cout, ks, stride, pad, 0, _ptr(x), ldx, _ptr(w), _ptr(None), 0,
               _ptr(out), ldo, _ptr(bias), _ptr(rowbias), ld_rb, _ptr(residual), ldr, 0, 1, _ptr(None), 0, _stream())
    return out
# ... 92 lines not shown
               _ptr(o), ldo, so, _ptr(do), lddo, sdo, _ptr(lse), _ptr(delta), _ptr(dq), lddq, sdq, _ptr(dk), lddk, sdk,
               _ptr(dv), lddv, sdv, _ptr(workspace(q.device).attn), workspace(q.device).attn.numel() * 4, int(parts), _stream())



def gn_scratch_floats(B, HW, C, G):
    return int(lib().raw("az_gn_scratch_floats")(B, HW, C, G))


def groupnorm_fwd(x, gamma, beta, y, stats, G, eps, silu):
    _req(x.dim() == 3 and y.shape == x.shape and x.stride(2) == 1 and y.stride(2) == 1, "groupnorm operands")
    B, HW, C = x.shape
    _req(x.stride(0) == HW * x.stride(1) and y.stride(0) == HW * y.stride(1), "batch stride")
    _req(stats.dtype == F32 and stats.numel() == B * G * 2 and stats.is_contiguous(), "stats")
    ws = workspace(x.device)
    _req(gn_scratch_floats(B, HW, C, G) <= ws.scratch.numel(), "scratch too small")
    with _prof('gn_fwd', 0.0, 4.0 * B * HW * C):
        lib().call("az_groupnorm_fwd", B, HW, C, G, float(eps), int(silu), _ptr(x), x.stride(1), _ptr(gamma), _ptr(beta),
               _ptr(y), y.stride(1), _ptr(stats), _ptr(ws.scratch), _stream())
    return y


def groupnorm_bwd(x, gamma, beta, stats, dy, dx, dgamma, dbeta, G, silu, accumulate_dx=False, dx_add=None):
    B, HW, C = x.shape
    if accumulate_dx and dx_add is None:
        dx_add = dx
    _req(dx_add is None or (dx is not None and dx_add.shape == x.shape and dx_add.stride(2) == 1 and dx_add.stride(0) == HW * dx_add.stride(1)), "dx_add layout")
    _req(dy.shape == x.shape and (dx is None or dx.shape == x.shape), "groupnorm bwd shapes")
    _req(x.stride(2) == 1 and dy.stride(2) == 1 and x.stride(0) == HW * x.stride(1) and dy.stride(0) == HW * dy.stride(1), "strides")
    ws = workspace(x.device)
    _req(gn_scratch_floats(B, HW, C, G) <= ws.scratch.numel(), "scratch too small")
    with _prof('gn_bwd', 0.0, 10.0 * B * HW * C):
        lib().call("az_groupnorm_bwd_ex", B, HW, C, G, int(silu), _ptr(x), x.stride(1), _ptr(gamma), _ptr(beta), _ptr(stats),
               _ptr(dy), dy.stride(1), _ptr(dx), dx.stride(1) if dx is not None else 0, _ptr(dx_add), dx_add.stride(1) if dx_add is not None else 0,
               _ptr(dgamma), _ptr(dbeta), _ptr(ws.scratch), _stream())


def layernorm_fwd(x, gamma, beta, y, stats, eps=1e-5):
    M, C, ldx = _rows(x)
    My, Cy, ldy = _rows(y)
    _req((M, C) == (My, Cy) and stats.dtype == F32 and stats.numel() == 2 * M, "layernorm operands")
    with _prof('ln_fwd', 0.0, 4.0 * M * C):
        lib().call("az_layernorm_fwd", M, C, float(eps), _ptr(x), ldx, _ptr(gamma), _ptr(beta), _ptr(y), ldy, _ptr(stats), _stream())
    return y


def layernorm_bwd(x, gamma, stats, dy, dx, dgamma, dbeta, accumulate_dx=False, dx_add=None):
    M, C, ldx = _rows(x)
    if accumulate_dx and dx_add is None:
        dx_add = dx
    ld_add = 0
    if dx_add is not None:
        Ma, Ca, ld_add = _rows(dx_add)
        _req(dx is not None and (Ma, Ca) == (M, C), "dx_add shape")
    _, _, lddy = _rows(dy)
    lddx = _rows(dx)[2] if dx is not None else 0
    ws = workspace(x.device)
    _req(int(lib().raw("az_ln_scratch_floats")(M, C)) <= ws.scratch.numel(), "scratch too small")
    with _prof('ln_bwd' if dx is not None else 'ln_bwd_param', 0.0, (8.0 if dx is not None else 4.0) * M * C):
        lib().call("az_layernorm_bwd_ex", M, C, _ptr(x), ldx, _ptr(gamma), _ptr(stats), _ptr(dy), lddy, _ptr(dx), lddx,
               _ptr(dx_add), ld_add, _ptr(dgamma), _ptr(dbeta), _ptr(ws.scratch), _stream())


def ln_partial_blocks(M: int) -> int:
    return int(lib().raw("az_ln_partial_blocks")(int(M)))


def layernorm_bwd_partial(x, gamma, stats, dy, dx, partial, dx_add=None, nblk=None):
    M, C, ldx = _rows(x)
    _, _, lddy = _rows(dy)
    _, _, lddx = _rows(dx)
    ld_add = 0
    if dx_add is not None:
        Ma, Ca, ld_add = _rows(dx_add)
        _req((Ma, Ca) == (M, C), "dx_add shape")
    if nblk is None:
        nblk = ln_partial_blocks(M)
    _req(partial.dtype == F32 and partial.is_contiguous() and partial.numel() >= nblk * C * 2, "partial buffer")
    with _prof('ln_bwd', 0.0, 8.0 * M * C):
        lib().call("az_layernorm_bwd_partial", M, C, _ptr(x), ldx, _ptr(gamma), _ptr(stats), _ptr(dy), lddy, _ptr(dx), lddx,
                   _ptr(dx_add), ld_add, _ptr(partial), int(nblk), _stream())


def ln_param_finish_multi(table, njobs: int, nblocks: int):
    with _prof('ln_bwd_param', 0.0, 0.0):
        lib().call("az_ln_param_finish_multi", _ptr(table), int(njobs), int(nblocks), _stream())



def geglu_fwd(proj, out):
    M, H2, ldp = _rows(proj)
    Mo, H, ldo = _rows(out)
    _req(Mo == M and H2 == 2 * H, "geglu shapes")
    with _prof('geglu_fwd', 0.0, 6.0 * M * H):
        lib().call("az_geglu_fwd", M, H, _ptr(proj), ldp, _ptr(out), ldo, _stream())
    return out


def geglu_bwd(proj, dout, dproj):
    M, H2, ldp = _rows(proj)
    _, H, lddo = _rows(dout)
    Md, Hd, lddp = _rows(dproj)
    _req(H2 == 2 * H and (Md, Hd) == (M, H2), "geglu bwd shapes")
    with _prof('geglu_bwd', 0.0, 10.0 * M * H):
        lib().call("az_geglu_bwd", M, H, _ptr(proj), ldp, _ptr(dout), lddo, _ptr(dproj), lddp, _stream())
    return dproj


def silu_fwd(x, y):
    _req(x.is_contiguous() and y.is_contiguous() and x.numel() == y.numel() and x.dtype == BF16, "silu operands")
    lib().call("az_silu_fwd", x.numel(), _ptr(x), _ptr(y), _stream())
    return y


def silu_bwd(x, dy, dx, accumulate=False):
    _req(x.is_contiguous() and dy.is_contiguous() and dx.is_contiguous() and x.numel() == dy.numel() == dx.numel(), "silu bwd")
    lib().call("az_silu_bwd", x.numel(), _ptr(x), _ptr(dy), _ptr(dx), int(accumulate), _stream())
    return dx


def add_rows(a, b, y):
    R, C, lda = _rows(a)
    Ry, Cy, ldy = _rows(y)
    _req((R, C) == (Ry, Cy), "add_rows shapes")
    ldb = 0
    if b is not None:
        Rb, Cb, ldb = _rows(b)
        _req((Rb, Cb) == (R, C), "add_rows b shape")
    with _prof('add_rows', 0.0, 6.0 * R * C):
        lib().call("az_add_rows", R, C, _ptr(a), lda, _ptr(b), ldb, _ptr(y), ldy, _stream())
    return y


def upsample2x_fwd(x, y):
    B, H, W, C = x.shape
    _req(x.is_contiguous() and y.is_contiguous() and tuple(y.shape) == (B, 2 * H, 2 * W, C) and x.dtype == BF16, "upsample")
    with _prof('upsample', 0.0, 10.0 * B * H * W * C):
        lib().call("az_upsample2x_fwd", B, H, W, C, _ptr(x), _ptr(y), _stream())
    return y


def upsample2x_bwd(dy, dx):
    B, H, W, C = dx.shape
    _req(dx.is_contiguous() and dy.is_contiguous() and tuple(dy.shape) == (B, 2 * H, 2 * W, C), "upsample bwd")
    with _prof('upsample', 0.0, 10.0 * B * H * W * C):
        lib().call("az_upsample2x_bwd", B, H, W, C, _ptr(dy), _ptr(dx), _stream())
    return dx


def colsum(x, rows_per_seg, out_f32):
    R, C, ldx = _rows(x)
    _req(R % rows_per_seg == 0 and out_f32.dtype == F32 and out_f32.numel() >= (R // rows_per_seg) * C, "colsum")
    ws = workspace(x.device)
    need = int(lib().raw("az_colsum_scratch_floats")(R, C, int(rows_per_seg)))
    half = ws.scratch.numel() // 2
    _req(need <= half, "colsum scratch too small")
    with _prof('colsum', 0.0, 2.0 * R * C):
        lib().call("az_colsum", R, C, int(rows_per_seg), _ptr(x), ldx, _ptr(out_f32), _ptr(ws.scratch[half:]), _stream())
    return out_f32


def colsum_grad(x, rows_per_seg, seg_out, bias_grad, n_real):
    R, C, ldx = _rows(x)
    _req(R % rows_per_seg == 0 and n_real <= C, "colsum_grad shapes")
    nseg = R // rows_per_seg
    if seg_out is not None:
# ... 94 lines not shown
```

aozora_sdxl_training_amd/tape.py:

```python
from __future__ import annotations

import ctypes
import struct

from ._lib import lib, AozoraError, ForkEvent, Call, Record, Wait, Live

OP_CALL, OP_EVENT_RECORD, OP_STREAM_WAIT, OP_BREAK = 0, 1, 2, 3


def _word(ty: str, a) -> int:
    if ty == "float":
        return struct.unpack("<I", struct.pack("<f", float(a)))[0]
    if hasattr(a, "value"):
        a = a.value
    if a is None:
        return 0
    return int(a)


_KERNEL_ENTRIES = frozenset({
    "az_spin", "az_gemm_bf16", "az_gemm_nt_grouped_bf16", "az_gemm_tn_grouped_bf16", "az_gemm_geglu_fwd_bf16", "az_gemm_wgrad_bias_bf16",
    "az_conv2d_bf16", "az_conv2d_wgrad_bias_bf16", "az_attn_fwd", "az_attn_bwd", "az_groupnorm_fwd", "az_groupnorm_bwd",
    "az_groupnorm_bwd_ex", "az_layernorm_fwd", "az_layernorm_bwd", "az_layernorm_bwd_ex", "az_layernorm_bwd_partial",
    "az_ln_param_finish_multi", "az_geglu_fwd", "az_geglu_bwd", "az_silu_fwd", "az_silu_bwd", "az_add_rows", "az_upsample2x_fwd",
    "az_upsample2x_bwd", "az_colsum", "az_colsum_grad", "az_reduce_segs_to_bf16", "az_transpose_bf16", "az_transpose_bf16_batched",
    "az_transpose_multi_bf16", "az_f32_to_bf16", "az_timestep_embed", "az_nchw_to_nhwc_pad", "az_nhwc_to_nchw", "az_noise_target",
    "az_mse_loss_fwd_bwd", "az_sumsq_bf16", "az_sumsq", "az_clip_coef", "az_adamw_flat", "az_adamw_flat_ex", "az_scale_bf16",
    "az_scale_f32", "az_stage_inputs", "az_adamw8bit_step"})
_NOT_KERNEL_ENTRIES = frozenset({"az_graph_begin", "az_graph_end", "az_graph_launch", "az_event_record", "az_stream_wait_event",
                                 "az_stream_sync", "az_memset_async", "az_memcpy_async", "az_titan_offload"})


def fuse_records(recorded, only_stream=None):
    stream_arg = {name: [i for i, (_, an) in enumerate(args) if an == "stream"] for name, (_, args) in lib().protos.items()}
    out, fused = [], 0
    last = {}
    last_rec = {}
    alias = {}
    for op in recorded:
        if isinstance(op, Call):
            idx = stream_arg.get(op.name)
            out.append([op, None])
            if not idx:
                last.clear(); last_rec.clear()
            else:
                st = _word("void*", op.args[idx[0]])
                last_rec.pop(st, None)
                if op.name not in _KERNEL_ENTRIES:
                    last.pop(st, None)
                else:
                    last[st] = len(out) - 1
        elif isinstance(op, Record):
            ev, st = op.event, op.stream.cuda_stream
            fork = isinstance(ev, ForkEvent)
            if fork and (only_stream is None or st == only_stream):
                if st in last_rec:
                    alias[id(ev)] = last_rec[st]
                    fused += 1
                    continue
                k = last.pop(st, None)
                if k is not None and out[k][1] is None:
                    out[k][1] = ev.cuda_event
                    last_rec[st] = ev
                    fused += 1
                    continue
            last.pop(st, None); last_rec.pop(st, None)
            if fork:
                last_rec[st] = ev
            out.append([op, None])
        elif isinstance(op, Wait):
            st = op.stream.cuda_stream
            out.append([Wait(op.stream, alias.get(id(op.event), op.event)), None])
            last.pop(st, None); last_rec.pop(st, None)
        else:
            out.append([op, None])
            last.clear(); last_rec.clear()
    flat = []
    for op, ev in out:
        if ev is None:
            flat.append(op)
        else:
            flat += [Call("az_set_launch_stop_event", (ctypes.c_void_p(ev),)), op, Call("az_set_launch_stop_event", (None,))]
    return flat, fused


def disarm_stop_event():
    lib()._fn["az_set_launch_stop_event"](None)


def issue(op):
    if isinstance(op, Call):
        rc = lib()._fn[op.name](*op.args)
        if rc:
            raise AozoraError(f"{op.name} failed with code {rc} while re-issuing the launch tape")
    elif isinstance(op, Record):
        op.event.record(op.stream)
    elif isinstance(op, Wait):
        op.event.wait(op.stream)
    else:
        op.fn(*op.args)


def replay(recorded):
    try:
        for op in recorded:
            issue(op)
    except BaseException:
        disarm_stop_event()
        raise


# ... 62 lines not shown
```

aozora_sdxl_training_amd/unet.py:

```python
from __future__ import annotations

import ctypes
import math
from dataclasses import dataclass
from types import SimpleNamespace
from typing import Dict, List, Optional, Tuple

import os
import torch

from . import ops
from ._lib import lib, AozoraError, ForkEvent, Record, Wait, Live
from .unet_spec import UNetConfig, SDXL_BASE, param_table, up_resnet_channels

@dataclass
class ExecPolicy:
    fork_events: bool = True
    fuse_records: int = 2
    side_batch: int = 1
    ln_fused: bool = True
    ln_defer: bool = True
    hoist: bool = True
    xkv_side: bool = True
    temb_side: bool = True
    geglu_fuse: bool = True
    cat_inplace: bool = True
    xkv_group: bool = True
    tn_group: int = 0
    host_tape: bool = True
    native_tape: bool = True
    side_streams: int = 1
    side_priority: int = 0
    main_priority: int = 0


BF16 = torch.bfloat16
F32 = torch.float32
ALIGN = 64


class Act:
    __slots__ = ("t", "g", "need_grad", "ready", "g_alias")

    def __init__(self, t: torch.Tensor, need_grad: bool = True):
        self.t = t
        self.g: Optional[torch.Tensor] = None
        self.need_grad = need_grad
        self.ready = None
        self.g_alias = False


class _Pool:

    def __init__(self, device):
        self.device = device
        self.bufs: List[torch.Tensor] = []
        self.cursor = 0

    def reset(self):
        self.cursor = 0

    def get(self, shape, dtype=BF16):
        if self.cursor < len(self.bufs):
            t = self.bufs[self.cursor]
            if tuple(t.shape) != tuple(shape) or t.dtype != dtype:
                raise AozoraError("activation pool replay mismatch (topology changed between steps)")
        else:
            t = torch.empty(shape, dtype=dtype, device=self.device)
            self.bufs.append(t)
        self.cursor += 1
        return t

    def nbytes(self):
        return sum(b.numel() * b.element_size() for b in self.bufs)


class _UNetCall(torch.autograd.Function):

    @staticmethod
    def forward(ctx, anchor, unet, sample, t_f32, ehs, pooled, tids_f32):
        B, C, H, W = sample.shape
        unet.begin_step((B, H, W, ehs.shape[1], "call"))
        x8 = unet._pool.get((B, H, W, 8), BF16)
        ops.nchw_to_nhwc_pad(sample.contiguous(), x8, C)
        pred = unet.forward_nhwc(x8, t_f32, ehs, pooled, tids_f32)
        out = torch.empty(B, unet.cfg.out_channels, H, W, dtype=BF16, device=sample.device)
        ops.nhwc_to_nchw(pred.t.view(B, H, W, unet.cfg.out_channels), out, unet.cfg.out_channels)
        ctx.unet, ctx.pred, ctx.geom = unet, pred, (B, H, W)
        return out

    @staticmethod
    def backward(ctx, grad_out):
        unet, (B, H, W) = ctx.unet, ctx.geom
        d8 = unet._pool.get((B, H, W, 8), BF16)
        g = grad_out.contiguous()
        if g.dtype not in (BF16, F32):
            g = g.float()
        ops.nchw_to_nhwc_pad(g, d8, unet.cfg.out_channels)
        unet.backward_nhwc(ctx.pred, d8)
        unet.expose_grads()
        return None, None, None, None, None, None, None


class AozoraUNet:
    def __init__(self, cfg: UNetConfig = SDXL_BASE, device="cuda:0", policy: Optional[ExecPolicy] = None):
        if not torch.cuda.is_available():
            raise AozoraError("AozoraUNet needs a HIP device; there is no CPU fallback")
        self.cfg = cfg
        self.policy = policy if policy is not None else ExecPolicy()
        self.config = SimpleNamespace(in_channels=cfg.in_channels, out_channels=cfg.out_channels,
                                      sample_size=128, cross_attention_dim=cfg.cross_attention_dim)
        self.device = torch.device(device)
        self._ctx = ctypes.c_void_p()
        if lib()._fn["az_init"](self.device.index if self.device.index is not None else torch.cuda.current_device(), ctypes.byref(self._ctx)):
            raise AozoraError("az_init failed")
        lib()._fn["az_make_current"](self._ctx)
        self.training = True
        self._table = param_table(cfg)
        self._layout()
        self._pools: Dict[tuple, _Pool] = {}
        self._pool: Optional[_Pool] = None
        self._tape: List = []
        self.conv_in = True
        self._anchor = torch.zeros((), device=self.device, requires_grad=True)
        self.concurrent_wgrad = True
        self._sides = [torch.cuda.Stream(device=self.device, priority=self.policy.side_priority)
                       for _ in range(max(1, self.policy.side_streams))]
        self._main_stream = None
        self._side_rr = 0
        self._side_q: List = []
        self._side_done = None
        self._ln_jobs: List = []
# ... 303 lines not shown
    def enable_gradient_checkpointing(self):
        return None

    def enable_xformers_memory_efficient_attention(self):
        return None

    def set_attn_processor(self, *_a, **_k):
        return None

    def to(self, device=None, *_a, **_k):
        if device is not None and torch.device(device).type != "cuda":
            raise AozoraError("AozoraUNet lives on a HIP device only")
        return self

    def train(self, mode=True):
        self.training = mode
        return self

    def requires_grad_(self, flag=True):
        for p in self._params.values():
            p.requires_grad = flag
        return self

    def _event(self):
        if self._ev_cursor == len(self._events):
            self._events.append(ForkEvent() if self.policy.fork_events else torch.cuda.Event())
        ev = self._events[self._ev_cursor]
        self._ev_cursor += 1
        return ev

    class _Side:

        def __init__(self, u):
            self.u = u

        def __enter__(self):
            u = self.u
            self.main = torch.cuda.current_stream()
            if not u.concurrent_wgrad:
                return self
            k = u._side_rr % len(u._sides)
            u._side_rr += 1
            self.stream = u._sides[k]
            ev = u._event(); u._ev_record(ev, self.main); u._st_wait(self.stream, ev)
            u._side_used = True
            self.ctx = torch.cuda.stream(self.stream); self.ctx.__enter__()
            ops.set_workspace_slot(1 + k)
            return self

        def __exit__(self, *a):
            u = self.u
            if not u.concurrent_wgrad:
                return False
            ops.set_workspace_slot(0)
            self.ctx.__exit__(*a)
            self.done = u._event(); u._ev_record(self.done, self.stream)
            return False

        done = None

        def join(self):
            if self.u.concurrent_wgrad and self.done is not None:
                self.u._st_wait(self.main, self.done)

    def _fork(self):
        return AozoraUNet._Side(self)

    def _trainable(self, name):
        return self._params[name].requires_grad

    def _new(self, rows, C, need_grad=True, dtype=BF16) -> Act:
        return Act(self._pool.get((rows, C), dtype), need_grad)

    def _wait_ready(self, a: Act):
        if a.ready is not None:
            self._st_wait(torch.cuda.current_stream(), a.ready)
            a.ready = None

    def _gbuf(self, a: Act):
        if a.g is None:
            a.g = self._pool.get(tuple(a.t.shape), BF16)
            a.g_alias = False
            return a.g, None
        if a.g_alias:
            old = a.g
            a.g = self._pool.get(tuple(a.t.shape), BF16)
            a.g_alias = False
            return a.g, old
        return a.g, a.g

    def _gbuf_single(self, a: Act, what: str):
        dst, add = self._gbuf(a)
        if add is not None:
            raise AozoraError(what + " must have a single consumer")
        return dst

    def _give_grad(self, a: Act, dy: torch.Tensor, alias=True):
        if not a.need_grad:
            return
        if a.g is None:
            a.g = dy
            a.g_alias = alias
        elif a.g_alias:
            old = a.g
            a.g = self._pool.get(tuple(a.t.shape), BF16)
            a.g_alias = False
            ops.add_rows(old, dy, a.g)
        else:
            ops.add_rows(a.g, dy, a.g)

    def _side_defer(self, fn):
        if not self.concurrent_wgrad:
            fn()
        else:
            self._side_q.append(fn)
            if len(self._side_q) >= self.policy.side_batch:
                self._flush_side()

    def _finish_ln_jobs(self):
        jobs, self._ln_jobs = self._ln_jobs, []
        if not jobs:
            return
        key = tuple(p.data_ptr() for p, _, _, _, _ in jobs)
        tab = self._ln_tables.get(key)
        if tab is None:
            rows_, blocks = [], 0
            for part, gw, gb, nblk, C in jobs:
                rows_.append([part.data_ptr(), gw.data_ptr() if gw is not None else 0, gb.data_ptr() if gb is not None else 0, nblk, C, blocks])
                blocks += (C + 31) // 32
            tab = (torch.tensor(rows_, dtype=torch.int64, device=self.device), len(rows_), blocks)
            self._ln_tables[key] = tab
        self._side_defer(lambda: ops.ln_param_finish_multi(tab[0], tab[1], tab[2]))

    @staticmethod
    def _linear_wgrad(dy, x, dW, bias_grad):
        ops.gemm(dy, x, dW, trans_a=True, trans_b=False, accumulate=True, split_k=0, bias_grad=bias_grad)

    def _queue_wgrads(self, jobs, grouped, tag=()):
        if not grouped:
            for job in jobs:
                self._side_defer(lambda job=job: self._linear_wgrad(*job))
            return
        key = tag + tuple((dy.data_ptr(), xt.data_ptr(), GW.data_ptr(), bg.data_ptr() if bg is not None else 0) for dy, xt, GW, bg in jobs)
        tab = self._tn_tables.get(key)
        if tab is None:
            tab = self._tn_tables[key] = ops.tn_group_table(jobs, self.device)
        self._side_defer(lambda: ops.gemm_tn_grouped(*tab))

    def _finish_tn_jobs(self):
        jobs, self._tn_jobs = self._tn_jobs, []
        if jobs:
            tiles = sum(((dy.shape[1] + 127) // 128) * ((xt.shape[1] + 127) // 128) for dy, xt, _, _ in jobs)
            self._queue_wgrads(jobs, tiles >= self.policy.tn_group)

    def _finish_xkv_jobs(self):
        jobs, self._xkv_jobs = self._xkv_jobs, []
        if jobs:
            self._queue_wgrads(jobs, len(jobs) > 1, ("xkv",))

    def _region_end(self):
        self._finish_ln_jobs()
        self._finish_tn_jobs()
        self._finish_xkv_jobs()
        self._flush_side()

    def _block_end(self):
        self._finish_tn_jobs()
        self._flush_side()

    def _flush_side(self):
        if not self._side_q:
            return self._side_done
        q, self._side_q = self._side_q, []
        side = self._fork()
        with side:
            for fn in q:
                fn()
        self._side_done = side.done
        return side.done

    def _bias_grad(self, dy: torch.Tensor, bname: Optional[str], n_real: int, rows_per_seg=None, seg_out: Optional[Act] = None):
        rows, C = dy.shape
        if seg_out is not None and seg_out.need_grad:
            if C != n_real:
                raise AozoraError("segment sums need an unpadded gradient")
            rps = rows_per_seg
        else:
            seg_out, rps = None, rows
        bias = self._gw[bname] if (bname is not None and self._trainable(bname)) else None
        if seg_out is None and bias is None:
            return
        ops.colsum_grad(dy, rps, seg_out.g.view(-1) if seg_out is not None else None, bias, n_real)

    def linear(self, x: Act, wname: str, bname: Optional[str], residual: Optional[Act] = None,
               w_override: Optional[Tuple[torch.Tensor, torch.Tensor, bool]] = None, out: Optional[Act] = None,
               pre: Optional[Act] = None, side_dgrad: bool = False, geglu_out: Optional[Act] = None) -> Act:
        if w_override is not None:
            W, GW, w_train = w_override
        else:
            W, GW, w_train = self._w[wname], self._gw[wname], self._trainable(wname)
        N = W.shape[0]
        WT = self._wt(W) if x.need_grad else None
        rows = x.t.shape[0]
        if pre is not None:
            y = pre
        else:
            y = out if out is not None else self._new(rows, N)
            if geglu_out is not None:
                ops.gemm_geglu_fwd(x.t, W, self._w[bname] if bname else None, y.t, geglu_out.t)
            else:
                ops.gemm(x.t, W, y.t, trans_b=True, bias=self._w[bname] if bname else None,
                         residual=residual.t if residual is not None else None,
                         split_k=0 if (rows <= 512 and residual is None) else 1)

        def bwd():
            dy = y.g
            if dy is None:
                return
            on_side = side_dgrad and self.policy.temb_side and self.concurrent_wgrad and len(self._sides) == 1
            if on_side:
                y.ready = None
            else:
                self._wait_ready(y)
            b_train = bname is not None and self._trainable(bname)
            job = (dy, x.t, GW, self._gw[bname] if b_train else None)

            def wgrad():
                if w_train:
                    self._linear_wgrad(*job)
                elif b_train:
                    self._bias_grad(dy, bname, N)
            if w_train and pre is not None and w_override is not None and rows <= 512 and self.policy.xkv_group and self.concurrent_wgrad and not on_side:
                self._xkv_jobs.append(job)
            elif w_train and self.policy.tn_group > 0 and 256 <= rows <= 8192 and not on_side:
                self._tn_jobs.append(job)
                if sum(((j[0].shape[1] + 127) // 128) * ((j[1].shape[1] + 127) // 128) for j in self._tn_jobs) >= self.policy.tn_group:
                    self._finish_tn_jobs()
            elif w_train or b_train:
                self._side_defer(wgrad)
            if x.need_grad:
                dx, add = self._gbuf(x)
                oop = add is not None and add is not dx

                def dgrad():
                    ops.gemm(dy, WT, dx, trans_b=True, accumulate=add is dx, residual=add if oop else None,
                             split_k=0 if (rows <= 512 and not oop) else 1)
                if on_side:
                    self._side_defer(dgrad)
                    x.ready = self._flush_side()
                else:
                    dgrad()
            if residual is not None:
                self._give_grad(residual, dy)
        self._tape.append(bwd)
        return y

    @staticmethod
    def _as3(t: torch.Tensor, B, HW):
        ld = t.stride(0)
        return t.as_strided((B, HW, t.shape[1]), (HW * ld, ld, 1))

    @staticmethod
    def _as4(t: torch.Tensor, B, H, W_):
        ld = t.stride(0)
        return t.as_strided((B, H, W_, t.shape[1]), (H * W_ * ld, W_ * ld, ld, 1))

    def conv(self, x: Act, geom, wname, bname, stride=1, rowbias: Optional[Act] = None, residual: Optional[Act] = None,
             upsample=False, out: Optional[Act] = None) -> Tuple[Act, tuple]:
        B, Hs, Ws = geom
        H, W_ = (2 * Hs, 2 * Ws) if upsample else (Hs, Ws)
        Wt = self._w[wname]
        Cout, ks, _, Cin = Wt.shape
        Ho = (H + 2 - 3) // stride + 1
        Wo = (W_ + 2 - 3) // stride + 1
        y = out if out is not None else self._new(B * Ho * Wo, Cout)
        if tuple(y.t.shape) != (B * Ho * Wo, Cout):
            raise AozoraError("conv destination shape")
        x4 = self._as4(x.t, B, Hs, Ws)
        ops.conv_fwd(x4, Wt, self._as4(y.t, B, Ho, Wo), stride=stride, bias=self._w[bname],
                     rowbias=rowbias.t if rowbias is not None else None,
                     residual=self._as4(residual.t, B, Ho, Wo) if residual is not None else None, upsample=upsample)

        def bwd():
            dy = y.g
            if dy is None:
                return
            dy4 = self._as4(dy, B, Ho, Wo)
            need_seg = rowbias is not None and rowbias.need_grad
            if need_seg:
                self._gbuf_single(rowbias, "segment-sum target")
            self._wait_ready(y)

            def wgrad():
                b_train = self._trainable(bname)
                fuse = self._trainable(wname) and (b_train or need_seg) and (not need_seg or ((Ho * Wo) % 64 == 0 and dy.shape[1] == Cout))
                if fuse:
                    ops.conv_wgrad(dy4, x4, self._gw[wname], stride=stride, cout_real=Cout, accumulate=True, split_k=0,
                                   bias_grad=self._gw[bname] if b_train else None,
                                   seg_grad=rowbias.g.view(-1) if need_seg else None, upsample=upsample)
                else:
                    if rowbias is not None or b_train:
                        self._bias_grad(dy, bname, Cout, rows_per_seg=Ho * Wo, seg_out=rowbias)
                    if self._trainable(wname):
                        ops.conv_wgrad(dy4, x4, self._gw[wname], stride=stride, cout_real=Cout, accumulate=True, split_k=0, upsample=upsample)
            self._side_defer(wgrad)
            if need_seg:
                rowbias.ready = self._flush_side()
            if x.need_grad:
                dx, add = self._gbuf(x)
                if upsample:
                    if add is not None:
                        raise AozoraError("upsample input must have a single consumer")
                    dxs = dx
                    dx = self._pool.get((B * H * W_, Cin), BF16)
                oop = add is not None and add is not dx
                res4 = self._as4(add, B, H, W_) if oop else None
                if Cout % 8 == 0 and dy.shape[1] == Cout:
                    o_w = (Wt.data_ptr() - self.pflat.data_ptr()) // 2
                    wt = self.wtflat[o_w:o_w + Wt.numel()].view(Cin, 3, 3, Cout)
                    ops.conv_dgrad_wt(dy4, wt, self._as4(dx, B, H, W_), stride=stride, accumulate=add is dx, residual=res4)
                else:
                    ops.conv_dgrad(dy4, Wt, self._as4(dx, B, H, W_), stride=stride, cout_real=Cout, accumulate=add is dx, residual=res4)
                if upsample:
                    ops.upsample2x_bwd(dx.view(B, H, W_, Cin), dxs.view(B, Hs, Ws, Cin))
            if residual is not None:
                self._give_grad(residual, dy)
        self._tape.append(bwd)
        return y, (B, Ho, Wo)

    def groupnorm(self, x: Act, geom, prefix, eps, silu) -> Act:
        B, H, W_ = geom
        C = x.t.shape[1]
        G = self.cfg.norm_groups
        y = self._new(B * H * W_, C)
        stats = self._pool.get((B * G * 2,), F32)
        gam, bet = self._w[prefix + ".weight"], self._w[prefix + ".bias"]
        x3 = self._as3(x.t, B, H * W_)
        ops.groupnorm_fwd(x3, gam, bet, y.t.view(B, H * W_, C), stats, G, eps, silu)

        def bwd():
            dy = y.g
            if dy is None:
                return
            tg, tb = self._trainable(prefix + ".weight"), self._trainable(prefix + ".bias")
            dy3 = self._as3(dy, B, H * W_)
            dx3, add3 = None, None
            if x.need_grad:
                dx, add = self._gbuf(x)
                dx3 = self._as3(dx, B, H * W_)
                if add is not None:
                    add3 = self._as3(add, B, H * W_)
            ops.groupnorm_bwd(x3, gam, bet, stats, dy3, dx3, self._gw[prefix + ".weight"] if tg else None,
                              self._gw[prefix + ".bias"] if tb else None, G, silu, dx_add=add3)
        self._tape.append(bwd)
        return y

    def layernorm(self, x: Act, prefix) -> Act:
        rows, C = x.t.shape
        y = self._new(rows, C)
        stats = self._pool.get((2 * rows,), F32)
        gam, bet = self._w[prefix + ".weight"], self._w[prefix + ".bias"]
        ops.layernorm_fwd(x.t, gam, bet, y.t, stats, 1e-5)

        def bwd():
            dy = y.g
            if dy is None:
                return
            dx, add = self._gbuf(x)
            gw = self._gw[prefix + ".weight"] if self._trainable(prefix + ".weight") else None
            gb = self._gw[prefix + ".bias"] if self._trainable(prefix + ".bias") else None
            self._wait_ready(y)
            if self.policy.ln_fused:
                if self.policy.ln_defer:
                    nblk = ops.ln_partial_blocks(rows)
                    part = self._pool.get((nblk * C * 2,), F32)
                if self.policy.ln_defer and (gw is not None or gb is not None):
                    ops.layernorm_bwd_partial(x.t, gam, stats, dy, dx, part, dx_add=add, nblk=nblk)
                    self._ln_jobs.append((part, gw, gb, nblk, C))
                    return
                ops.layernorm_bwd(x.t, gam, stats, dy, dx, gw, gb, dx_add=add)
                return
            if gw is not None or gb is not None:
                self._side_defer(lambda: ops.layernorm_bwd(x.t, gam, stats, dy, None, gw, gb))
            ops.layernorm_bwd(x.t, gam, stats, dy, dx, None, None, dx_add=add)
        self._tape.append(bwd)
        return y

    def silu(self, x: Act) -> Act:
        y = self._new(*x.t.shape)
        ops.silu_fwd(x.t, y.t)

        def bwd():
            if y.g is None:
                return
            self._wait_ready(y)
            dx, add = self._gbuf(x)
            if add is not None and add is not dx:
                raise AozoraError("SiLU input gradient cannot be accumulated out of place")
            ops.silu_bwd(x.t, y.g, dx, accumulate=add is dx)
        self._tape.append(bwd)
        return y

    def _fused_w(self, names: List[str]):
        o0, st0, _ = self._slots[names[0]]
        rows, cols = 0, st0[1]
        off = o0
        for n in names:
            o, st, _ = self._slots[n]
            if o != off or st[1] != cols or math.prod(st) % ALIGN:
                raise AozoraError(f"parameters {names} are not adjacent in the flat buffer")
            rows += st[0]
            off += math.prod(st)
        W = self.pflat[o0:off].view(rows, cols)
        G = self.gflat[o0:off].view(rows, cols)
        return W, G, any(self._trainable(n) for n in names)

    def attention(self, x: Act, B, T, prefix, ctx: Optional[Act], ctx_len, residual: Act) -> Act:
        C = x.t.shape[1]
        heads = C // self.cfg.head_dim
        scale = 1.0 / math.sqrt(self.cfg.head_dim)
        if ctx is None:
            qkv = self.linear(x, None, None, w_override=self._fused_w([prefix + ".to_q.weight", prefix + ".to_k.weight", prefix + ".to_v.weight"]))
            q3 = qkv.t.view(B, T, 3 * C)[..., :C]
            k3 = qkv.t.view(B, T, 3 * C)[..., C:2 * C]
            v3 = qkv.t.view(B, T, 3 * C)[..., 2 * C:]
            Tk, kv_train = T, True
        else:
            q = self.linear(x, prefix + ".to_q.weight", None)
            kv_w = self._fused_w([prefix + ".to_k.weight", prefix + ".to_v.weight"])
            kv_train = kv_w[2]
            kv = self.linear(ctx, None, None, w_override=kv_w, pre=self._hoisted.pop(prefix + ".kv", None))
            q3 = q.t.view(B, T, C)
            k3 = kv.t.view(B, ctx_len, 2 * C)[..., :C]
            v3 = kv.t.view(B, ctx_len, 2 * C)[..., C:]
            Tk = ctx_len
        o = self._new(B * T, C)
        lse = self._pool.get((B * heads * T,), F32)
        ops.attn_fwd(q3, k3, v3, o.t.view(B, T, C), lse, heads, scale)

        def bwd():
            do = o.g
            if do is None:
                return
            delta = self._pool.get((B * heads * T,), F32)
            if ctx is None:
                dqkv = self._gbuf_single(qkv, "attention projections")
                d3 = dqkv.view(B, T, 3 * C)
                dq3, dk3, dv3 = d3[..., :C], d3[..., C:2 * C], d3[..., 2 * C:]
            else:
                dq = self._gbuf_single(q, "attention projections")
                dkv = self._gbuf_single(kv, "attention projections")
                dq3 = dq.view(B, T, C)
                dk3, dv3 = dkv.view(B, ctx_len, 2 * C)[..., :C], dkv.view(B, ctx_len, 2 * C)[..., C:]
            o3, do3 = o.t.view(B, T, C), do.view(B, T, C)
# ... 306 lines not shown
```

include/aozora_hip.h:

```cpp
#ifndef AOZORA_HIP_H
#define AOZORA_HIP_H
#ifdef __cplusplus
extern "C" {
#endif

int az_version(void);
int az_device_info(int* out3);
int az_graph_begin(void* stream);
int az_graph_end(void* stream, void** graph_exec_out);
int az_graph_launch(void* graph_exec, void* stream);
int az_graph_destroy(void* graph_exec);
int az_host_alloc(void** ptr_host, long bytes);
int az_host_free(void* ptr_host);
int az_event_create(void** ev);
int az_event_record(void* ev, void* stream);
int az_event_sync(void* ev);
int az_event_elapsed_ms(void* ev_start, void* ev_stop, float* ms);
int az_event_destroy(void* ev);
int az_event_create_fork(void** ev);
int az_stream_wait_event(void* stream, void* ev);
int az_set_launch_stop_event(void* ev);
int az_stream_sync(void* stream);
int az_spin(long microseconds, void* stream);
int az_memset_async(void* ptr, int value, long bytes, void* stream);
int az_memcpy_async(void* dst, const void* src, long bytes, int kind, void* stream);

int az_gemm_set_tile(int bm, int bn);
int az_gemm_set_tile_ex(int bm, int bn, int waves);
int az_gemm_set_exclusive(int on);
int az_set_option(const char* name, int value);
int az_get_option(const char* name, int* value);
int az_init(int device, void** handle);
int az_make_current(void* handle);
int az_context_device(void* handle, int* device);
int az_destroy(void* handle);
int az_gemm_bf16(int transA, int transB, int M, int N, int K, const void* A, long lda, const void* B, long ldb,
                 void* C, long ldc, const void* bias, const void* rowbias, int rows_per_seg, long ld_rowbias,
                 const void* residual, long ldr, int accumulate, int split_k, void* workspace, long workspace_bytes,
                 void* stream);

int az_gemm_nt_grouped_bf16(int M, int K, const void* A, long lda, const void* groups_dev, int ngroups, long total_tiles_n, void* stream);

int az_gemm_tn_grouped_bf16(const void* groups_dev, int ngroups, long total_tiles, void* stream);

int az_gemm_geglu_fwd_bf16(int M, int H, int K, const void* X, long lda, const void* W, long ldb, const void* bias, void* proj, long ldp,
                           void* out, long ldo, void* stream);

int az_gemm_wgrad_bias_bf16(int M, int N, int K, const void* dY, long lddy, const void* X, long ldx, void* dW, long lddw,
                            int accumulate, int split_k, void* workspace, long workspace_bytes, void* bias_grad, int n_real,
                            void* stream);

int az_conv2d_bf16(int mode, int batch, int Hin, int Win, int Cin, int Hout, int Wout, int Cout, int ksize, int stride,
                   int pad, int cpad, const void* X, long ldx, const void* W, const void* dY, long lddy, void* out,
                   long ldo, const void* bias, const void* rowbias, long ld_rowbias, const void* residual, long ldr,
                   int accumulate, int split_k, void* workspace, long workspace_bytes, void* stream);
int az_conv2d_wgrad_bias_bf16(int batch, int Hin, int Win, int Cin, int Hout, int Wout, int Cout, int ksize, int stride, int pad,
                              const void* X, long ldx, const void* dY, long lddy, void* dW, int accumulate, int split_k,
                              void* workspace, long workspace_bytes, void* bias_grad, void* seg_grad, void* stream);

int az_attn_fwd(int batch, int heads, int Tq, int Tk, float scale, const void* Q, long ldq, long sq, const void* K,
                long ldk, long sk, const void* V, long ldv, long sv, void* O, long ldo, long so, void* lse,
                void* stream);
int az_attn_bwd(int batch, int heads, int Tq, int Tk, float scale, const void* Q, long ldq, long sq, const void* K,
                long ldk, long sk, const void* V, long ldv, long sv, const void* O, long ldo, long so, const void* dO,
                long lddo, long sdo, const void* lse, void* delta, void* dQ, long lddq, long sdq, void* dK, long lddk,
                long sdk, void* dV, long lddv, long sdv, void* workspace, long workspace_bytes, int parts, void* stream);

long az_gn_scratch_floats(int batch, int HW, int C, int G);
int az_groupnorm_fwd(int batch, int HW, int C, int G, float eps, int fuse_silu, const void* x, long ldx,
                     const void* gamma, const void* beta, void* y, long ldy, void* stats, void* partial, void* stream);
int az_groupnorm_bwd(int batch, int HW, int C, int G, int fuse_silu, const void* x, long ldx, const void* gamma,
                     const void* beta, const void* stats, const void* dy, long lddy, void* dx, long lddx,
                     int accumulate_dx, void* dgamma, void* dbeta, void* partial, void* stream);
int az_groupnorm_bwd_ex(int batch, int HW, int C, int G, int fuse_silu, const void* x, long ldx, const void* gamma,
                        const void* beta, const void* stats, const void* dy, long lddy, void* dx, long lddx,
                        const void* dx_add, long ld_add, void* dgamma, void* dbeta, void* partial, void* stream);
long az_ln_scratch_floats(int M, int C);
int az_layernorm_fwd(int M, int C, float eps, const void* x, long ldx, const void* gamma, const void* beta, void* y,
                     long ldy, void* stats, void* stream);
int az_layernorm_bwd(int M, int C, const void* x, long ldx, const void* gamma, const void* stats, const void* dy,
                     long lddy, void* dx, long lddx, int accumulate_dx, void* dgamma, void* dbeta, void* partial,
                     void* stream);
int az_layernorm_bwd_ex(int M, int C, const void* x, long ldx, const void* gamma, const void* stats, const void* dy,
                        long lddy, void* dx, long lddx, const void* dx_add, long ld_add, void* dgamma, void* dbeta, void* partial,
                        void* stream);
int az_layernorm_bwd_partial(int M, int C, const void* x, long ldx, const void* gamma, const void* stats, const void* dy,
                             long lddy, void* dx, long lddx, const void* dx_add, long ld_add, void* partial, int nblk, void* stream);
int az_ln_partial_blocks(int M);
int az_ln_param_finish_multi(const void* jobs_dev, int njobs, long nblocks, void* stream);

int az_geglu_fwd(int M, int H, const void* proj, long ldp, void* out, long ldo, void* stream);
int az_geglu_bwd(int M, int H, const void* proj, long ldp, const void* dout, long lddo, void* dproj, long lddp,
                 void* stream);
int az_silu_fwd(long n, const void* x, void* y, void* stream);
int az_silu_bwd(long n, const void* x, const void* dy, void* dx, int accumulate, void* stream);
int az_add_rows(long rows, int C, const void* a, long lda, const void* b, long ldb, void* y, long ldy, void* stream);
int az_upsample2x_fwd(int batch, int H, int W, int C, const void* x, void* y, void* stream);
int az_upsample2x_bwd(int batch, int H, int W, int C, const void* dy, void* dx, void* stream);
long az_colsum_scratch_floats(long rows, int C, int rows_per_seg);
int az_colsum(long rows, int C, int rows_per_seg, const void* x, long ldx, void* out_f32, void* scratch_f32, void* stream);
int az_colsum_grad(long rows, int C, int rows_per_seg, const void* x, long ldx, void* seg_out_bf16, void* bias_grad_bf16,
                   int n_real, void* scratch_f32, void* stream);
int az_reduce_segs_to_bf16(int nseg, int n, const void* src_f32, void* dst, int accumulate, void* stream);
int az_transpose_bf16(int R, int C, const void* src, long ld_src, void* dst, long ld_dst, void* stream);
int az_transpose_bf16_batched(int batch, int R, int C, const void* src, long ld_src, long bstride_src, void* dst, long ld_dst,
                              long bstride_dst, void* stream);
int az_transpose_multi_bf16(const void* jobs_dev, int njobs, long ntiles, void* stream);
int az_f32_to_bf16(long n, const void* src, void* dst, void* stream);
int az_timestep_embed(int n, int dim, const void* t_f32, void* out, long ldo, void* stream);
int az_nchw_to_nhwc_pad(int batch, int C, int HW, int Cpad, const void* src, int src_is_f32, void* dst, void* stream);
int az_nhwc_to_nchw(int batch, int C, int HW, int ldsrc, const void* src, void* dst, int dst_is_f32, void* stream);

int az_noise_target(int mode, int batch, int C, int HW, int cpad, const void* latents, const void* noise,
                    const void* coef_a, const void* coef_b, void* noisy_nhwc, void* target_f32, void* stream);
int az_mse_loss_fwd_bwd(int batch, int C, int HW, const void* pred, long ldp, const void* target_f32, const void* w,
                        float grad_scale, void* loss_out, void* per_sample_out, void* dpred, int cpad, void* scratch_f32,
                        void* stream);

int az_sumsq_bf16(long n, const void* g, void* out_f32, int accumulate, void* scratch_f32, void* stream);
int az_sumsq(long n, const void* g, int dtype, void* out_f32, int accumulate, void* scratch_f32, void* stream);
int az_clip_coef(const void* sumsq_f32, float max_norm, float grad_unscale, void* coef_f32, void* norm_f32, void* stream);
int az_adamw_flat(long n, void* p, const void* g, void* m, void* v, int mdtype, const void* hyper, const void* coef,
                  void* stream);
int az_raven_step(long n, void* p, const void* g, void* m_host, void* v_host, int mdtype, const void* hyper,
                  const void* coef, void* staging, long chunk_elems, void* stream_compute, void* stream_h2d,
                  void* stream_d2h);
int az_adamw_flat_ex(long n, void* p, const void* g, int gdtype, void* m, void* v, int mdtype, const void* hyper,
                     const void* coef, void* stream);
int az_raven_step_ex(long n, void* p, const void* g, int gdtype, void* m_host, void* v_host, int mdtype, const void* hyper,
                     const void* coef, void* staging, long chunk_elems, void* stream_compute, void* stream_h2d,
                     void* stream_d2h);
int az_scale_bf16(long n, void* g, const void* coef_f32, void* stream);
int az_scale_f32(long n, void* x, const void* coef_f32, void* stream);
int az_stage_inputs(int nseg, const void* src_ptrs, const void* dst_ptrs, const void* seg_bytes, int ncoef, const void* coef_host,
                    void* coef_dev, void* stream);
int az_titan_offload(long n, const void* g, void* g_host_f32, void* staging_f32, int accumulate, void* stream);
int az_adamw8bit_step(int ntensors, const void* desc, long nblocks, const void* hyper, const void* qmaps, const void* coef,
                      void* stream);

int az_tape_fn_id(const char* name);
int az_tape_create(void** tape);
int az_tape_destroy(void* tape);
int az_tape_add(void* tape, int kind, int fn, const void* words, int nwords);
long az_tape_play(void* tape, long start);
int az_tape_last_error(void* tape, long* index, int* rc);

#ifdef __cplusplus
}
#endif
#endif
```

Measured before the change: 1.058 iters/sec.

## Fold split-K slab reduction of LN-input data gradient into LayerNorm backward

When a big-K NT data-gradient GEMM feeding a LayerNorm output would use split-K, the GEMM now writes raw fp32 slabs and the LayerNorm backward kernel sums those slabs itself while computing dx. This removes the separate split-K reduction pass and the bf16 round trip of the intermediate gradient. In exchange it adds a new slab-reading kernel variant, tightens ordering constraints on the workspace (it checks that no launch comes in between), and applies only when the activation has a single gradient contributor on the main stream.

```diff
diff --git a/aozora_sdxl_training_amd/_lib.py b/aozora_sdxl_training_amd/_lib.py
--- a/aozora_sdxl_training_amd/_lib.py
+++ b/aozora_sdxl_training_amd/_lib.py
@@ -74,9 +74,12 @@
             fn.argtypes = [_CTYPES[t] for t, _ in args]
             self._fn[name] = fn
         self.recorder = None
+        self.ncalls = 0
 
     def call(self, name: str, *args):
         fn = self._fn[name]
+        if not name.startswith("az_event_"):
+            self.ncalls += 1
         rc = fn(*args)
         if rc != 0:
             raise AozoraError(f"{name} failed with code {rc}" + (" (argument error)" if rc <= -1000 else " (HIP error)"))
diff --git a/aozora_sdxl_training_amd/csrc/az_common.h b/aozora_sdxl_training_amd/csrc/az_common.h
--- a/aozora_sdxl_training_amd/csrc/az_common.h
+++ b/aozora_sdxl_training_amd/csrc/az_common.h
@@ -131,6 +131,7 @@
   AZ_OPT_GN_RPT,
   AZ_OPT_GN_RPT_BWD,
   AZ_OPT_GN_RPT_APPLY,
+  AZ_OPT_NT_SLAB_MINK,
   AZ_OPT_COUNT
 };
 int az_opt(int id);
diff --git a/aozora_sdxl_training_amd/csrc/az_gemm.hip b/aozora_sdxl_training_amd/csrc/az_gemm.hip
--- a/aozora_sdxl_training_amd/csrc/az_gemm.hip
+++ b/aozora_sdxl_training_amd/csrc/az_gemm.hip
@@ -1145,6 +1145,24 @@
   p.tiles_m = (p.M + 255) / 256; p.tiles_n = (p.N + bn - 1) / bn;
 }
 
+int nt_big_split_choice(int M, int N, int K, long ws_bytes, int mink, int& bn_out) {
+  const int sb = az_opt(AZ_OPT_LDS_EXCLUSIVE) ? az_opt(AZ_OPT_NT_SPLIT_FWD) : az_opt(AZ_OPT_NT_SPLIT_BIG);
+  if (sb <= 1 || g_force_bm || (K % BK) != 0 || K < mink || (N & 7)) return 0;
+  const int kt = K / BK;
+  double best = 0.0; int bs = 0;
+  for (int bn = 256; bn <= 320; bn += 64) {
+    if (bn == 320 && ((N % 320) || !az_opt(AZ_OPT_GEMM8))) continue;
+    const long tl = (long)((M + 255) / 256) * ((N + bn - 1) / bn);
+    if (tl > 128) continue;
+    for (int sp = 2; sp <= sb; ++sp) {
+      if (kt / sp < 8 || tl * sp > 256 || (long)sp * M * N * 4 > ws_bytes) break;
+      const double score = (double)(tl * sp) / 256.0 - 0.02 * (sp - 1);
+      if (score > best + 1e-9) { best = score; bs = sp; bn_out = bn; }
+    }
+  }
+  return (bs > 1 && best >= 0.7) ? bs : 0;
+}
+
 }
 
 extern "C" {
@@ -1205,25 +1223,12 @@
     p.cs_bias = (bf16_t*)bias_grad; p.cs_n_real = n_real; p.cs_seg_out = nullptr;
   }
   bool big_split = false; int split_bn = 256;
-  {
-    const int sb = az_opt(AZ_OPT_LDS_EXCLUSIVE) ? az_opt(AZ_OPT_NT_SPLIT_FWD) : az_opt(AZ_OPT_NT_SPLIT_BIG);
-    if (sb > 1 && !transA && transB && !g_force_bm && !rowbias && workspace && (K % BK) == 0 && K >= az_opt(AZ_OPT_NT_SPLIT_MINK) &&
-        (split_k == 0 || split_k == 1) && (!residual || (((ldr & 7) == 0) && (((uintptr_t)residual & 15) == 0))) &&
-        ((N & 7) == 0) && ((ldc & 7) == 0) && (((uintptr_t)C & 15) == 0) && (((uintptr_t)workspace & 15) == 0)) {
-      const int kt = K / BK;
-      double best = 0.0; int bs = 0;
-      for (int bn = 256; bn <= 320; bn += 64) {
-        if (bn == 320 && ((N % 320) || !az_opt(AZ_OPT_GEMM8))) continue;
-        const long tl = (long)((M + 255) / 256) * ((N + bn - 1) / bn);
-        if (tl > 128) continue;
-        for (int sp = 2; sp <= sb; ++sp) {
-          if (kt / sp < 8 || tl * sp > 256 || (long)sp * M * N * 4 > workspace_bytes) break;
-          const double score = (double)(tl * sp) / 256.0 - 0.02 * (sp - 1);
-          if (score > best + 1e-9) { best = score; bs = sp; split_bn = bn; }
-        }
-      }
-      if (bs > 1 && best >= 0.7) { big_split = true; split_k = bs; }
-    }
+  if (!transA && transB && !rowbias && workspace && (split_k == 0 || split_k == 1) &&
+      (!residual || (((ldr & 7) == 0) && (((uintptr_t)residual & 15) == 0))) &&
+      ((ldc & 7) == 0) && (((uintptr_t)C & 15) == 0) && (((uintptr_t)workspace & 15) == 0)) {
+    int bn = 256;
+    const int bs = nt_big_split_choice(M, N, K, workspace_bytes, az_opt(AZ_OPT_NT_SPLIT_MINK), bn);
+    if (bs > 1) { big_split = true; split_k = bs; split_bn = bn; }
   }
   if (!big_split && !transA && transB && !g_force_bm && !rowbias && !residual && workspace && (K % BK) == 0 && (split_k == 0 || split_k == 1) &&
       !az_opt(AZ_OPT_LDS_EXCLUSIVE) && az_opt(AZ_OPT_TILE_POLICY) < 5) {
@@ -1254,6 +1259,33 @@
                  void* stream) {
   return gemm_impl(transA, transB, M, N, K, A, lda, B, ldb, C, ldc, bias, rowbias, rows_per_seg, ld_rowbias, residual, ldr,
                    accumulate, split_k, workspace, workspace_bytes, nullptr, 0, stream);
+}
+
+int az_gemm_nt_split_plan(int M, int N, int K, long workspace_bytes, int* splits, int* bn) {
+  if (!splits || !bn) return AZ_ERR_ARG(76);
+  *splits = 0; *bn = 0;
+  if (M <= 0 || N <= 0 || K <= 0 || workspace_bytes < 0) return AZ_ERR_ARG(76);
+  if (az_opt(AZ_OPT_INKERNEL_FINISH) && workspace_bytes >= TICKET_BYTES + 65536 && !(workspace_bytes & 15)) workspace_bytes -= TICKET_BYTES;
+  int w = 256;
+  const int s = nt_big_split_choice(M, N, K, workspace_bytes, az_opt(AZ_OPT_NT_SLAB_MINK), w);
+  if (s > 1) { *splits = s; *bn = w; }
+  return AZ_OK;
+}
+
+int az_gemm_nt_slabs_bf16(int M, int N, int K, const void* A, long lda, const void* B, long ldb, int splits, int bn,
+                          void* workspace, long workspace_bytes, void* stream) {
+  if (M <= 0 || N <= 0 || K <= 0 || (N & 7) || (K % BK) != 0) return AZ_ERR_ARG(77);
+  if ((lda & 7) || (ldb & 7) || ((uintptr_t)A & 15) || ((uintptr_t)B & 15) || !A || !B) return AZ_ERR_ARG(78);
+  if (splits < 2 || splits > 8 || (bn != 256 && bn != 320) || (bn == 320 && (N % 320))) return AZ_ERR_ARG(79);
+  if (!workspace || ((uintptr_t)workspace & 15) || (long)splits * M * N * 4 > workspace_bytes || (long)splits * M * N * 4 >= 0x7FFFFFF0L) return AZ_ERR_ARG(80);
+  Params p{};
+  p.A = (const bf16_t*)A; p.B = (const bf16_t*)B; p.lda = lda; p.ldb = ldb; p.M = M; p.N = N; p.K = K;
+  p.C = nullptr; p.ldc = N; p.ws = (float*)workspace;
+  choose_split(p, splits, workspace_bytes, false, true, true);
+  if (p.ksplit != splits) return AZ_ERR_ARG(81);
+  apply_gemm8(p, bn);
+  if (p.bn != bn) return AZ_ERR_ARG(81);
+  return launch<A_ROW, B_NT>(p, (hipStream_t)stream);
 }
 
 int az_gemm_geglu_fwd_bf16(int M, int H, int K, const void* X, long lda, const void* W, long ldb, const void* bias, void* proj, long ldp,
diff --git a/aozora_sdxl_training_amd/csrc/az_norm.hip b/aozora_sdxl_training_amd/csrc/az_norm.hip
--- a/aozora_sdxl_training_amd/csrc/az_norm.hip
+++ b/aozora_sdxl_training_amd/csrc/az_norm.hip
@@ -393,13 +393,15 @@
   }
 }
 
-template <int NCH>
-__global__ __launch_bounds__(256) void ln_bwd_fused_kernel(int M, int C, int rows_per_block, const bf16_t* __restrict__ x, long ldx,
+template <int NCH, bool SLAB = false>
+__global__ __launch_bounds__(256) __attribute__((amdgpu_waves_per_eu(SLAB && NCH <= 3 ? 2 : 1)))
+void ln_bwd_fused_kernel(int M, int C, int rows_per_block, const bf16_t* __restrict__ x, long ldx,
                                  const bf16_t* __restrict__ gamma, const float* __restrict__ stats, const bf16_t* __restrict__ dy,
-                                 long lddy, bf16_t* dx, long lddx, const bf16_t* dadd, long ldadd, float* __restrict__ partial) {
+                                 long lddy, bf16_t* dx, long lddx, const bf16_t* dadd, long ldadd, float* __restrict__ partial,
+                                 const float* __restrict__ slabs, int nslab) {
   const bool accumulate = dadd != nullptr;
   extern __shared__ float sh[];
-  const int lane = threadIdx.x & 63, w = threadIdx.x >> 6;
+  const int lane = threadIdx.x & 63, w = __builtin_amdgcn_readfirstlane(threadIdx.x >> 6);
   const int cch = C >> 3;
   const int r0 = blockIdx.x * rows_per_block;
   int r1 = r0 + rows_per_block; if (r1 > M) r1 = M;
@@ -413,21 +415,48 @@
     for (int e = 0; e < 8; ++e) { pg[i][e] = 0.f; pb[i][e] = 0.f; }
   }
   const float invC = 1.0f / (float)C;
+  unsigned coff[NCH];
+#pragma unroll
+  for (int i = 0; i < NCH; ++i) coff[i] = lane + 64 * i < cch ? (unsigned)(lane + 64 * i) * 8u : 0u;
   uint4 nx[NCH], nd[NCH], np[NCH];
   float nmean = 0.f, nrstd = 0.f;
+  const long slab_pitch = (long)M * C;
   auto fetch = [&](int row) {
     nmean = stats[row * 2]; nrstd = stats[row * 2 + 1];
+    const bf16_t* xr = x + (long)row * ldx;
+    const bf16_t* dr = SLAB ? nullptr : dy + (long)row * lddy;
+    const bf16_t* ar = accumulate ? dadd + (long)row * ldadd : nullptr;
 #pragma unroll
     for (int i = 0; i < NCH; ++i) {
       const int cc = lane + 64 * i;
       if (cc < cch) {
-        nx[i] = *reinterpret_cast<const uint4*>(x + (long)row * ldx + cc * 8);
-        nd[i] = *reinterpret_cast<const uint4*>(dy + (long)row * lddy + cc * 8);
-        if (accumulate) np[i] = *reinterpret_cast<const uint4*>(dadd + (long)row * ldadd + cc * 8);
+        nx[i] = *reinterpret_cast<const uint4*>(xr + coff[i]);
+        if constexpr (!SLAB) nd[i] = *reinterpret_cast<const uint4*>(dr + coff[i]);
+        if (accumulate) np[i] = *reinterpret_cast<const uint4*>(ar + coff[i]);
       }
     }
   };
-  if (r0 + w < r1) fetch(r0 + w);
+  auto fold = [&](int row) {
+    if constexpr (SLAB) {
+      const float* base = slabs + (long)row * C;
+      float4 na[NCH][2];
+#pragma unroll
+      for (int i = 0; i < NCH; ++i) { na[i][0] = *reinterpret_cast<const float4*>(base + coff[i]); na[i][1] = *reinterpret_cast<const float4*>(base + coff[i] + 4); }
+      auto add = [](float4& s, const float4& v) { s.x += v.x; s.y += v.y; s.z += v.z; s.w += v.w; };
+      for (int z = 1; z < nslab; ++z) {
+        const float* sp = base + (long)z * slab_pitch;
+        float4 a[NCH][2];
+#pragma unroll
+        for (int i = 0; i < NCH; ++i) { a[i][0] = *reinterpret_cast<const float4*>(sp + coff[i]); a[i][1] = *reinterpret_cast<const float4*>(sp + coff[i] + 4); }
+#pragma unroll
+        for (int i = 0; i < NCH; ++i) { add(na[i][0], a[i][0]); add(na[i][1], a[i][1]); }
+      }
+#pragma unroll
+      for (int i = 0; i < NCH; ++i)
+        nd[i] = make_uint4(pack2bf(na[i][0].x, na[i][0].y), pack2bf(na[i][0].z, na[i][0].w), pack2bf(na[i][1].x, na[i][1].y), pack2bf(na[i][1].z, na[i][1].w));
+    }
+  };
+  if (r0 + w < r1) { fetch(r0 + w); fold(r0 + w); }
   for (int row = r0 + w; row < r1; row += 4) {
     const float mean = nmean, rstd = nrstd;
     uint4 cx[NCH], cd[NCH], prev[NCH];
@@ -463,20 +492,23 @@
           float vv = rstd * (dg[i][e] - c1 - xh[i][e] * c2);
           o[e] = accumulate ? o[e] + vv : vv;
         }
-        *reinterpret_cast<uint4*>(dx + (long)row * lddx + cc * 8) = pack8(o);
+        *reinterpret_cast<uint4*>(dx + (long)row * lddx + coff[i]) = pack8(o);
       }
     }
+    if (SLAB && row + 4 < r1) fold(row + 4);
   }
   float* out = partial + (long)blockIdx.x * C * 2;
+  int tid = threadIdx.x;
+  if constexpr (SLAB) asm volatile("" : "+v"(tid));
 #pragma unroll
   for (int i = 0; i < NCH; ++i) {
     if (i) __syncthreads();
-    float* d = sh + ((long)w * 64 + lane) * 16;
+    float* d = sh + (long)tid * 16;
 #pragma unroll
     for (int e = 0; e < 8; e += 2)
       *reinterpret_cast<float4*>(d + e * 2) = make_float4(pg[i][e], pb[i][e], pg[i][e + 1], pb[i][e + 1]);
     __syncthreads();
-    const int l2 = threadIdx.x >> 2, q = threadIdx.x & 3;
+    const int l2 = tid >> 2, q = tid & 3;
     const int cc = l2 + 64 * i;
     if (cc < cch) {
       float4 a = *reinterpret_cast<const float4*>(sh + (long)l2 * 16 + q * 4);
@@ -700,7 +732,7 @@
     const int rpb = ((M + nblk - 1) / nblk + 3) / 4 * 4;
     const size_t shb = (size_t)4 * 64 * 16 * sizeof(float);
 #define LN_FU(N) az_launch(ln_bwd_fused_kernel<N>, dim3(nblk), b1, shb, st, M, C, rpb, (const bf16_t*)x, ldx, (const bf16_t*)gamma, \
-                                    (const float*)stats, (const bf16_t*)dy, lddy, (bf16_t*)dx, lddx, (const bf16_t*)dx_add, ld_add, (float*)partial)
+                                    (const float*)stats, (const bf16_t*)dy, lddy, (bf16_t*)dx, lddx, (const bf16_t*)dx_add, ld_add, (float*)partial, (const float*)nullptr, 0)
     if (nch == 1) LN_FU(1); else if (nch == 2) LN_FU(2); else if (nch == 3) LN_FU(3); else LN_FU(4);
 #undef LN_FU
     AZ_CHECK_LAUNCH();
@@ -749,7 +781,26 @@
   const int nch = (C / 8 + 63) / 64;
   const size_t shb = (size_t)4 * 64 * 16 * sizeof(float);
 #define LN_FU(N) az_launch(ln_bwd_fused_kernel<N>, dim3(nblk), dim3(256), shb, st, M, C, rpb, (const bf16_t*)x, ldx, (const bf16_t*)gamma, \
-                                    (const float*)stats, (const bf16_t*)dy, lddy, (bf16_t*)dx, lddx, (const bf16_t*)dx_add, ld_add, (float*)partial)
+                                    (const float*)stats, (const bf16_t*)dy, lddy, (bf16_t*)dx, lddx, (const bf16_t*)dx_add, ld_add, (float*)partial, (const float*)nullptr, 0)
+  if (nch == 1) LN_FU(1); else if (nch == 2) LN_FU(2); else if (nch == 3) LN_FU(3); else LN_FU(4);
+#undef LN_FU
+  AZ_CHECK_LAUNCH();
+  return AZ_OK;
+}
+
+int az_layernorm_bwd_partial_slabs(int M, int C, const void* x, long ldx, const void* gamma, const void* stats, const void* slabs, int splits,
+                                   void* dx, long lddx, const void* dx_add, long ld_add, void* partial, int nblk, void* stream) {
+  if (M <= 0 || (C & 7) || C > 64 * 8 * LN_MAXCH || (ldx & 7) || !dx || (lddx & 7) || (dx_add && (ld_add & 7)) || !partial) return AZ_ERR_ARG(32);
+  if (splits < 2 || splits > 8 || !slabs || ((uintptr_t)slabs & 15)) return AZ_ERR_ARG(35);
+  if (nblk <= 0 || nblk > LN_FUSED_MAX_BLOCKS) return AZ_ERR_ARG(34);
+  const int rpb = ((M + nblk - 1) / nblk + 3) / 4 * 4;
+  if ((M + rpb - 1) / rpb != nblk) return AZ_ERR_ARG(34);
+  hipStream_t st = (hipStream_t)stream;
+  const int nch = (C / 8 + 63) / 64;
+  const size_t shb = (size_t)4 * 64 * 16 * sizeof(float);
+#define LN_FU(N) az_launch((ln_bwd_fused_kernel<N, true>), dim3(nblk), dim3(256), shb, st, M, C, rpb, (const bf16_t*)x, ldx, (const bf16_t*)gamma, \
+                                    (const float*)stats, (const bf16_t*)nullptr, 0L, (bf16_t*)dx, lddx, (const bf16_t*)dx_add, ld_add, (float*)partial, \
+                                    (const float*)slabs, splits)
   if (nch == 1) LN_FU(1); else if (nch == 2) LN_FU(2); else if (nch == 3) LN_FU(3); else LN_FU(4);
 #undef LN_FU
   AZ_CHECK_LAUNCH();
diff --git a/aozora_sdxl_training_amd/csrc/az_runtime.hip b/aozora_sdxl_training_amd/csrc/az_runtime.hip
--- a/aozora_sdxl_training_amd/csrc/az_runtime.hip
+++ b/aozora_sdxl_training_amd/csrc/az_runtime.hip
@@ -9,7 +9,7 @@
 struct OptDef { const char* name; int def; };
 const OptDef OPT_DEFS[AZ_OPT_COUNT] = {
   {"TILE_POLICY", 4}, {"BIG_FILL", 5}, {"SPLIT_SLOTS", 384}, {"NOSPLIT_TILES", 256}, {"LDS_EXCLUSIVE", 0}, {"NT_SPLIT_BIG", 3},
-  {"NT_SPLIT_MINK", 5120}, {"ATTN_SPLIT_TARGET", 384}, {"LN_RPB", 32}, {"INKERNEL_FINISH", 0}, {"NT_SPLIT2_MINK", 0}, {"GEMM_ABLATE", 0}, {"GEMM8", 1}, {"NT_SPLIT_FWD", 0}, {"ATTN_PIPE", 15}, {"XCD_SPLIT", 1}, {"ATTN_XCD", 15}, {"NORM_STAT_BF16", 1}, {"GN_RPT", 4}, {"GN_RPT_BWD", 32}, {"GN_RPT_APPLY", 32},
+  {"NT_SPLIT_MINK", 5120}, {"ATTN_SPLIT_TARGET", 384}, {"LN_RPB", 32}, {"INKERNEL_FINISH", 0}, {"NT_SPLIT2_MINK", 0}, {"GEMM_ABLATE", 0}, {"GEMM8", 1}, {"NT_SPLIT_FWD", 0}, {"ATTN_PIPE", 15}, {"XCD_SPLIT", 1}, {"ATTN_XCD", 15}, {"NORM_STAT_BF16", 1}, {"GN_RPT", 4}, {"GN_RPT_BWD", 32}, {"GN_RPT_APPLY", 32}, {"NT_SLAB_MINK", 5120},
 };
 std::atomic<int> g_opt[AZ_OPT_COUNT];
 std::once_flag g_opt_once;
diff --git a/aozora_sdxl_training_amd/csrc/az_tape_dispatch.inc b/aozora_sdxl_training_amd/csrc/az_tape_dispatch.inc
--- a/aozora_sdxl_training_amd/csrc/az_tape_dispatch.inc
+++ b/aozora_sdxl_training_amd/csrc/az_tape_dispatch.inc
@@ -20,6 +20,7 @@
   "az_gemm_bf16",
   "az_gemm_geglu_fwd_bf16",
   "az_gemm_nt_grouped_bf16",
+  "az_gemm_nt_slabs_bf16",
   "az_gemm_set_exclusive",
   "az_gemm_set_tile",
   "az_gemm_set_tile_ex",
@@ -35,6 +36,7 @@
   "az_layernorm_bwd",
   "az_layernorm_bwd_ex",
   "az_layernorm_bwd_partial",
+  "az_layernorm_bwd_partial_slabs",
   "az_layernorm_fwd",
   "az_ln_param_finish_multi",
   "az_ln_partial_blocks",
@@ -68,7 +70,7 @@
   "az_upsample2x_fwd",
   "az_version",
 };
-static const int AZ_TAPE_FN_NARGS[] = {7, 9, 10, 9, 35, 19, 6, 8, 10, 29, 22, 1, 1, 2, 1, 4, 9, 7, 22, 13, 8, 1, 2, 3, 4, 16, 1, 1, 2, 19, 20, 15, 1, 15, 16, 15, 11, 4, 1, 1, 5, 4, 14, 8, 8, 12, 13, 14, 6, 4, 4, 1, 6, 4, 2, 8, 1, 2, 7, 6, 6, 6, 7, 10, 4, 7, 7, 0};
+static const int AZ_TAPE_FN_NARGS[] = {7, 9, 10, 9, 35, 19, 6, 8, 10, 29, 22, 1, 1, 2, 1, 4, 9, 7, 22, 13, 8, 12, 1, 2, 3, 4, 16, 1, 1, 2, 19, 20, 15, 1, 15, 16, 15, 15, 11, 4, 1, 1, 5, 4, 14, 8, 8, 12, 13, 14, 6, 4, 4, 1, 6, 4, 2, 8, 1, 2, 7, 6, 6, 6, 7, 10, 4, 7, 7, 0};
 static int az_tape_dispatch(int fn, const long* w) {
   switch (fn) {
     case 0: return az_adamw8bit_step((int)w[0], (const void*)w[1], (long)w[2], (const void*)w[3], (const void*)w[4], (const void*)w[5], (void*)w[6]);
@@ -92,53 +94,55 @@
     case 18: return az_gemm_bf16((int)w[0], (int)w[1], (int)w[2], (int)w[3], (int)w[4], (const void*)w[5], (long)w[6], (const void*)w[7], (long)w[8], (void*)w[9], (long)w[10], (const void*)w[11], (const void*)w[12], (int)w[13], (long)w[14], (const void*)w[15], (long)w[16], (int)w[17], (int)w[18], (void*)w[19], (long)w[20], (void*)w[21]);
     case 19: return az_gemm_geglu_fwd_bf16((int)w[0], (int)w[1], (int)w[2], (const void*)w[3], (long)w[4], (const void*)w[5], (long)w[6], (const void*)w[7], (void*)w[8], (long)w[9], (void*)w[10], (long)w[11], (void*)w[12]);
     case 20: return az_gemm_nt_grouped_bf16((int)w[0], (int)w[1], (const void*)w[2], (long)w[3], (const void*)w[4], (int)w[5], (long)w[6], (void*)w[7]);
-    case 21: return az_gemm_set_exclusive((int)w[0]);
-    case 22: return az_gemm_set_tile((int)w[0], (int)w[1]);
-    case 23: return az_gemm_set_tile_ex((int)w[0], (int)w[1], (int)w[2]);
-    case 24: return az_gemm_tn_grouped_bf16((const void*)w[0], (int)w[1], (long)w[2], (void*)w[3]);
-    case 25: return az_gemm_wgrad_bias_bf16((int)w[0], (int)w[1], (int)w[2], (const void*)w[3], (long)w[4], (const void*)w[5], (long)w[6], (void*)w[7], (long)w[8], (int)w[9], (int)w[10], (void*)w[11], (long)w[12], (void*)w[13], (int)w[14], (void*)w[15]);
-    case 26: return az_graph_begin((void*)w[0]);
-    case 27: return az_graph_destroy((void*)w[0]);
-    case 28: return az_graph_launch((void*)w[0], (void*)w[1]);
-    case 29: return az_groupnorm_bwd((int)w[0], (int)w[1], (int)w[2], (int)w[3], (int)w[4], (const void*)w[5], (long)w[6], (const void*)w[7], (const void*)w[8], (const void*)w[9], (const void*)w[10], (long)w[11], (void*)w[12], (long)w[13], (int)w[14], (void*)w[15], (void*)w[16], (void*)w[17], (void*)w[18]);
-    case 30: return az_groupnorm_bwd_ex((int)w[0], (int)w[1], (int)w[2], (int)w[3], (int)w[4], (const void*)w[5], (long)w[6], (const void*)w[7], (const void*)w[8], (const void*)w[9], (const void*)w[10], (long)w[11], (void*)w[12], (long)w[13], (const void*)w[14], (long)w[15], (void*)w[16], (void*)w[17], (void*)w[18], (void*)w[19]);
-    case 31: return az_groupnorm_fwd((int)w[0], (int)w[1], (int)w[2], (int)w[3], word_float(w[4]), (int)w[5], (const void*)w[6], (long)w[7], (const void*)w[8], (const void*)w[9], (void*)w[10], (long)w[11], (void*)w[12], (void*)w[13], (void*)w[14]);
-    case 32: return az_host_free((void*)w[0]);
-    case 33: return az_layernorm_bwd((int)w[0], (int)w[1], (const void*)w[2], (long)w[3], (const void*)w[4], (const void*)w[5], (const void*)w[6], (long)w[7], (void*)w[8], (long)w[9], (int)w[10], (void*)w[11], (void*)w[12], (void*)w[13], (void*)w[14]);
-    case 34: return az_layernorm_bwd_ex((int)w[0], (int)w[1], (const void*)w[2], (long)w[3], (const void*)w[4], (const void*)w[5], (const void*)w[6], (long)w[7], (void*)w[8], (long)w[9], (const void*)w[10], (long)w[11], (void*)w[12], (void*)w[13], (void*)w[14], (void*)w[15]);
-    case 35: return az_layernorm_bwd_partial((int)w[0], (int)w[1], (const void*)w[2], (long)w[3], (const void*)w[4], (const void*)w[5], (const void*)w[6], (long)w[7], (void*)w[8], (long)w[9], (const void*)w[10], (long)w[11], (void*)w[12], (int)w[13], (void*)w[14]);
-    case 36: return az_layernorm_fwd((int)w[0], (int)w[1], word_float(w[2]), (const void*)w[3], (long)w[4], (const void*)w[5], (const void*)w[6], (void*)w[7], (long)w[8], (void*)w[9], (void*)w[10]);
-    case 37: return az_ln_param_finish_multi((const void*)w[0], (int)w[1], (long)w[2], (void*)w[3]);
-    case 38: return az_ln_partial_blocks((int)w[0]);
-    case 39: return az_make_current((void*)w[0]);
-    case 40: return az_memcpy_async((void*)w[0], (const void*)w[1], (long)w[2], (int)w[3], (void*)w[4]);
-    case 41: return az_memset_async((void*)w[0], (int)w[1], (long)w[2], (void*)w[3]);
-    case 42: return az_mse_loss_fwd_bwd((int)w[0], (int)w[1], (int)w[2], (const void*)w[3], (long)w[4], (const void*)w[5], (const void*)w[6], word_float(w[7]), (void*)w[8], (void*)w[9], (void*)w[10], (int)w[11], (void*)w[12], (void*)w[13]);
-    case 43: return az_nchw_to_nhwc_pad((int)w[0], (int)w[1], (int)w[2], (int)w[3], (const void*)w[4], (int)w[5], (void*)w[6], (void*)w[7]);
-    case 44: return az_nhwc_to_nchw((int)w[0], (int)w[1], (int)w[2], (int)w[3], (const void*)w[4], (void*)w[5], (int)w[6], (void*)w[7]);
-    case 45: return az_noise_target((int)w[0], (int)w[1], (int)w[2], (int)w[3], (int)w[4], (const void*)w[5], (const void*)w[6], (const void*)w[7], (const void*)w[8], (void*)w[9], (void*)w[10], (void*)w[11]);
-    case 46: return az_raven_step((long)w[0], (void*)w[1], (const void*)w[2], (void*)w[3], (void*)w[4], (int)w[5], (const void*)w[6], (const void*)w[7], (void*)w[8], (long)w[9], (void*)w[10], (void*)w[11], (void*)w[12]);
-    case 47: return az_raven_step_ex((long)w[0], (void*)w[1], (const void*)w[2], (int)w[3], (void*)w[4], (void*)w[5], (int)w[6], (const void*)w[7], (const void*)w[8], (void*)w[9], (long)w[10], (void*)w[11], (void*)w[12], (void*)w[13]);
-    case 48: return az_reduce_segs_to_bf16((int)w[0], (int)w[1], (const void*)w[2], (void*)w[3], (int)w[4], (void*)w[5]);
-    case 49: return az_scale_bf16((long)w[0], (void*)w[1], (const void*)w[2], (void*)w[3]);
-    case 50: return az_scale_f32((long)w[0], (void*)w[1], (const void*)w[2], (void*)w[3]);
-    case 51: return az_set_launch_stop_event((void*)w[0]);
-    case 52: return az_silu_bwd((long)w[0], (const void*)w[1], (const void*)w[2], (void*)w[3], (int)w[4], (void*)w[5]);
-    case 53: return az_silu_fwd((long)w[0], (const void*)w[1], (void*)w[2], (void*)w[3]);
-    case 54: return az_spin((long)w[0], (void*)w[1]);
-    case 55: return az_stage_inputs((int)w[0], (const void*)w[1], (const void*)w[2], (const void*)w[3], (int)w[4], (const void*)w[5], (void*)w[6], (void*)w[7]);
-    case 56: return az_stream_sync((void*)w[0]);
-    case 57: return az_stream_wait_event((void*)w[0], (void*)w[1]);
-    case 58: return az_sumsq((long)w[0], (const void*)w[1], (int)w[2], (void*)w[3], (int)w[4], (void*)w[5], (void*)w[6]);
-    case 59: return az_sumsq_bf16((long)w[0], (const void*)w[1], (void*)w[2], (int)w[3], (void*)w[4], (void*)w[5]);
-    case 60: return az_timestep_embed((int)w[0], (int)w[1], (const void*)w[2], (void*)w[3], (long)w[4], (void*)w[5]);
-    case 61: return az_titan_offload((long)w[0], (const void*)w[1], (void*)w[2], (void*)w[3], (int)w[4], (void*)w[5]);
-    case 62: return az_transpose_bf16((int)w[0], (int)w[1], (const void*)w[2], (long)w[3], (void*)w[4], (long)w[5], (void*)w[6]);
-    case 63: return az_transpose_bf16_batched((int)w[0], (int)w[1], (int)w[2], (const void*)w[3], (long)w[4], (long)w[5], (void*)w[6], (long)w[7], (long)w[8], (void*)w[9]);
-    case 64: return az_transpose_multi_bf16((const void*)w[0], (int)w[1], (long)w[2], (void*)w[3]);
-    case 65: return az_upsample2x_bwd((int)w[0], (int)w[1], (int)w[2], (int)w[3], (const void*)w[4], (void*)w[5], (void*)w[6]);
-    case 66: return az_upsample2x_fwd((int)w[0], (int)w[1], (int)w[2], (int)w[3], (const void*)w[4], (void*)w[5], (void*)w[6]);
-    case 67: return az_version();
+    case 21: return az_gemm_nt_slabs_bf16((int)w[0], (int)w[1], (int)w[2], (const void*)w[3], (long)w[4], (const void*)w[5], (long)w[6], (int)w[7], (int)w[8], (void*)w[9], (long)w[10], (void*)w[11]);
+    case 22: return az_gemm_set_exclusive((int)w[0]);
+    case 23: return az_gemm_set_tile((int)w[0], (int)w[1]);
+    case 24: return az_gemm_set_tile_ex((int)w[0], (int)w[1], (int)w[2]);
+    case 25: return az_gemm_tn_grouped_bf16((const void*)w[0], (int)w[1], (long)w[2], (void*)w[3]);
+    case 26: return az_gemm_wgrad_bias_bf16((int)w[0], (int)w[1], (int)w[2], (const void*)w[3], (long)w[4], (const void*)w[5], (long)w[6], (void*)w[7], (long)w[8], (int)w[9], (int)w[10], (void*)w[11], (long)w[12], (void*)w[13], (int)w[14], (void*)w[15]);
+    case 27: return az_graph_begin((void*)w[0]);
+    case 28: return az_graph_destroy((void*)w[0]);
+    case 29: return az_graph_launch((void*)w[0], (void*)w[1]);
+    case 30: return az_groupnorm_bwd((int)w[0], (int)w[1], (int)w[2], (int)w[3], (int)w[4], (const void*)w[5], (long)w[6], (const void*)w[7], (const void*)w[8], (const void*)w[9], (const void*)w[10], (long)w[11], (void*)w[12], (long)w[13], (int)w[14], (void*)w[15], (void*)w[16], (void*)w[17], (void*)w[18]);
+    case 31: return az_groupnorm_bwd_ex((int)w[0], (int)w[1], (int)w[2], (int)w[3], (int)w[4], (const void*)w[5], (long)w[6], (const void*)w[7], (const void*)w[8], (const void*)w[9], (const void*)w[10], (long)w[11], (void*)w[12], (long)w[13], (const void*)w[14], (long)w[15], (void*)w[16], (void*)w[17], (void*)w[18], (void*)w[19]);
+    case 32: return az_groupnorm_fwd((int)w[0], (int)w[1], (int)w[2], (int)w[3], word_float(w[4]), (int)w[5], (const void*)w[6], (long)w[7], (const void*)w[8], (const void*)w[9], (void*)w[10], (long)w[11], (void*)w[12], (void*)w[13], (void*)w[14]);
+    case 33: return az_host_free((void*)w[0]);
+    case 34: return az_layernorm_bwd((int)w[0], (int)w[1], (const void*)w[2], (long)w[3], (const void*)w[4], (const void*)w[5], (const void*)w[6], (long)w[7], (void*)w[8], (long)w[9], (int)w[10], (void*)w[11], (void*)w[12], (void*)w[13], (void*)w[14]);
+    case 35: return az_layernorm_bwd_ex((int)w[0], (int)w[1], (const void*)w[2], (long)w[3], (const void*)w[4], (const void*)w[5], (const void*)w[6], (long)w[7], (void*)w[8], (long)w[9], (const void*)w[10], (long)w[11], (void*)w[12], (void*)w[13], (void*)w[14], (void*)w[15]);
+    case 36: return az_layernorm_bwd_partial((int)w[0], (int)w[1], (const void*)w[2], (long)w[3], (const void*)w[4], (const void*)w[5], (const void*)w[6], (long)w[7], (void*)w[8], (long)w[9], (const void*)w[10], (long)w[11], (void*)w[12], (int)w[13], (void*)w[14]);
+    case 37: return az_layernorm_bwd_partial_slabs((int)w[0], (int)w[1], (const void*)w[2], (long)w[3], (const void*)w[4], (const void*)w[5], (const void*)w[6], (int)w[7], (void*)w[8], (long)w[9], (const void*)w[10], (long)w[11], (void*)w[12], (int)w[13], (void*)w[14]);
+    case 38: return az_layernorm_fwd((int)w[0], (int)w[1], word_float(w[2]), (const void*)w[3], (long)w[4], (const void*)w[5], (const void*)w[6], (void*)w[7], (long)w[8], (void*)w[9], (void*)w[10]);
+    case 39: return az_ln_param_finish_multi((const void*)w[0], (int)w[1], (long)w[2], (void*)w[3]);
+    case 40: return az_ln_partial_blocks((int)w[0]);
+    case 41: return az_make_current((void*)w[0]);
+    case 42: return az_memcpy_async((void*)w[0], (const void*)w[1], (long)w[2], (int)w[3], (void*)w[4]);
+    case 43: return az_memset_async((void*)w[0], (int)w[1], (long)w[2], (void*)w[3]);
+    case 44: return az_mse_loss_fwd_bwd((int)w[0], (int)w[1], (int)w[2], (const void*)w[3], (long)w[4], (const void*)w[5], (const void*)w[6], word_float(w[7]), (void*)w[8], (void*)w[9], (void*)w[10], (int)w[11], (void*)w[12], (void*)w[13]);
+    case 45: return az_nchw_to_nhwc_pad((int)w[0], (int)w[1], (int)w[2], (int)w[3], (const void*)w[4], (int)w[5], (void*)w[6], (void*)w[7]);
+    case 46: return az_nhwc_to_nchw((int)w[0], (int)w[1], (int)w[2], (int)w[3], (const void*)w[4], (void*)w[5], (int)w[6], (void*)w[7]);
+    case 47: return az_noise_target((int)w[0], (int)w[1], (int)w[2], (int)w[3], (int)w[4], (const void*)w[5], (const void*)w[6], (const void*)w[7], (const void*)w[8], (void*)w[9], (void*)w[10], (void*)w[11]);
+    case 48: return az_raven_step((long)w[0], (void*)w[1], (const void*)w[2], (void*)w[3], (void*)w[4], (int)w[5], (const void*)w[6], (const void*)w[7], (void*)w[8], (long)w[9], (void*)w[10], (void*)w[11], (void*)w[12]);
+    case 49: return az_raven_step_ex((long)w[0], (void*)w[1], (const void*)w[2], (int)w[3], (void*)w[4], (void*)w[5], (int)w[6], (const void*)w[7], (const void*)w[8], (void*)w[9], (long)w[10], (void*)w[11], (void*)w[12], (void*)w[13]);
+    case 50: return az_reduce_segs_to_bf16((int)w[0], (int)w[1], (const void*)w[2], (void*)w[3], (int)w[4], (void*)w[5]);
+    case 51: return az_scale_bf16((long)w[0], (void*)w[1], (const void*)w[2], (void*)w[3]);
+    case 52: return az_scale_f32((long)w[0], (void*)w[1], (const void*)w[2], (void*)w[3]);
+    case 53: return az_set_launch_stop_event((void*)w[0]);
+    case 54: return az_silu_bwd((long)w[0], (const void*)w[1], (const void*)w[2], (void*)w[3], (int)w[4], (void*)w[5]);
+    case 55: return az_silu_fwd((long)w[0], (const void*)w[1], (void*)w[2], (void*)w[3]);
+    case 56: return az_spin((long)w[0], (void*)w[1]);
+    case 57: return az_stage_inputs((int)w[0], (const void*)w[1], (const void*)w[2], (const void*)w[3], (int)w[4], (const void*)w[5], (void*)w[6], (void*)w[7]);
+    case 58: return az_stream_sync((void*)w[0]);
+    case 59: return az_stream_wait_event((void*)w[0], (void*)w[1]);
+    case 60: return az_sumsq((long)w[0], (const void*)w[1], (int)w[2], (void*)w[3], (int)w[4], (void*)w[5], (void*)w[6]);
+    case 61: return az_sumsq_bf16((long)w[0], (const void*)w[1], (void*)w[2], (int)w[3], (void*)w[4], (void*)w[5]);
+    case 62: return az_timestep_embed((int)w[0], (int)w[1], (const void*)w[2], (void*)w[3], (long)w[4], (void*)w[5]);
+    case 63: return az_titan_offload((long)w[0], (const void*)w[1], (void*)w[2], (void*)w[3], (int)w[4], (void*)w[5]);
+    case 64: return az_transpose_bf16((int)w[0], (int)w[1], (const void*)w[2], (long)w[3], (void*)w[4], (long)w[5], (void*)w[6]);
+    case 65: return az_transpose_bf16_batched((int)w[0], (int)w[1], (int)w[2], (const void*)w[3], (long)w[4], (long)w[5], (void*)w[6], (long)w[7], (long)w[8], (void*)w[9]);
+    case 66: return az_transpose_multi_bf16((const void*)w[0], (int)w[1], (long)w[2], (void*)w[3]);
+    case 67: return az_upsample2x_bwd((int)w[0], (int)w[1], (int)w[2], (int)w[3], (const void*)w[4], (void*)w[5], (void*)w[6]);
+    case 68: return az_upsample2x_fwd((int)w[0], (int)w[1], (int)w[2], (int)w[3], (const void*)w[4], (void*)w[5], (void*)w[6]);
+    case 69: return az_version();
     default: return AZ_ERR_ARG(60);
   }
 }
diff --git a/aozora_sdxl_training_amd/ops.py b/aozora_sdxl_training_amd/ops.py
--- a/aozora_sdxl_training_amd/ops.py
+++ b/aozora_sdxl_training_amd/ops.py
@@ -147,6 +147,29 @@
     return out
 
 
+def gemm_nt_split_plan(M: int, N: int, K: int, device=None):
+    ws = workspace(device)
+    s, bn = ctypes.c_int(), ctypes.c_int()
+    rc = lib()._fn["az_gemm_nt_split_plan"](int(M), int(N), int(K), ws.splitk.numel() * 4, ctypes.byref(s), ctypes.byref(bn))
+    if rc:
+        raise AozoraError(f"az_gemm_nt_split_plan failed with code {rc}")
+    return s.value, bn.value
+
+
+def gemm_nt_slabs(a, b, splits: int, bn: int):
+    M, K, lda = _rows(a)
+    N, Kb, ldb = _rows(b)
+    _req(K == Kb, f"K mismatch {K} vs {Kb}")
+    _req(lda % 8 == 0 and ldb % 8 == 0 and a.data_ptr() % 16 == 0 and b.data_ptr() % 16 == 0, "A/B layout")
+    _req(N % 8 == 0 and K % 64 == 0, "slab product: N % 8 == 0 and K % 64 == 0")
+    ws = workspace(a.device)
+    _req(2 <= splits <= 8 and splits * M * N <= ws.splitk.numel(), "slab product: split count / workspace size")
+    with _prof("gemm_nt" + (f" {M}x{N}x{K} slabs" if PROFILE_SHAPES else ""), 2.0 * M * N * K, 2.0 * (M * K + N * K) + 4.0 * splits * M * N):
+        lib().call("az_gemm_nt_slabs_bf16", M, N, K, _ptr(a), lda, _ptr(b), ldb, int(splits), int(bn), _ptr(ws.splitk),
+                   ws.splitk.numel() * 4, _stream())
+    return ws.splitk[:splits * M * N].view(splits, M, N)
+
+
 def gemm_nt_grouped(a, table, ngroups: int, total_tiles_n: int, sum_n: int = 0):
     M, K, lda = _rows(a)
     _req(K % 8 == 0 and lda % 8 == 0 and a.data_ptr() % 16 == 0, "grouped gemm: A layout")
@@ -405,6 +428,24 @@
                    _ptr(dx_add), ld_add, _ptr(partial), int(nblk), _stream())
 
 
+def layernorm_bwd_partial_slabs(x, gamma, stats, slabs, dx, partial, dx_add=None, nblk=None):
+    M, C, ldx = _rows(x)
+    _, _, lddx = _rows(dx)
+    _req(slabs.is_cuda and slabs.dtype == F32 and slabs.dim() == 3 and slabs.is_contiguous() and tuple(slabs.shape[1:]) == (M, C),
+         "slabs must be contiguous fp32 [splits][M][C]")
+    splits = slabs.shape[0]
+    ld_add = 0
+    if dx_add is not None:
+        Ma, Ca, ld_add = _rows(dx_add)
+        _req((Ma, Ca) == (M, C), "dx_add shape")
+    if nblk is None:
+        nblk = ln_partial_blocks(M)
+    _req(partial.dtype == F32 and partial.is_contiguous() and partial.numel() >= nblk * C * 2, "partial buffer")
+    with _prof('ln_bwd', 0.0, (6.0 + 4.0 * splits) * M * C):
+        lib().call("az_layernorm_bwd_partial_slabs", M, C, _ptr(x), ldx, _ptr(gamma), _ptr(stats), _ptr(slabs), int(splits),
+                   _ptr(dx), lddx, _ptr(dx_add), ld_add, _ptr(partial), int(nblk), _stream())
+
+
 def ln_param_finish_multi(table, njobs: int, nblocks: int):
     with _prof('ln_bwd_param', 0.0, 0.0):
         lib().call("az_ln_param_finish_multi", _ptr(table), int(njobs), int(nblocks), _stream())
diff --git a/aozora_sdxl_training_amd/tape.py b/aozora_sdxl_training_amd/tape.py
--- a/aozora_sdxl_training_amd/tape.py
+++ b/aozora_sdxl_training_amd/tape.py
@@ -26,7 +26,7 @@
     "az_upsample2x_bwd", "az_colsum", "az_colsum_grad", "az_reduce_segs_to_bf16", "az_transpose_bf16", "az_transpose_bf16_batched",
     "az_transpose_multi_bf16", "az_f32_to_bf16", "az_timestep_embed", "az_nchw_to_nhwc_pad", "az_nhwc_to_nchw", "az_noise_target",
     "az_mse_loss_fwd_bwd", "az_sumsq_bf16", "az_sumsq", "az_clip_coef", "az_adamw_flat", "az_adamw_flat_ex", "az_scale_bf16",
-    "az_scale_f32", "az_stage_inputs", "az_adamw8bit_step"})
+    "az_scale_f32", "az_stage_inputs", "az_adamw8bit_step", "az_gemm_nt_slabs_bf16", "az_layernorm_bwd_partial_slabs"})
 _NOT_KERNEL_ENTRIES = frozenset({"az_graph_begin", "az_graph_end", "az_graph_launch", "az_event_record", "az_stream_wait_event",
                                  "az_stream_sync", "az_memset_async", "az_memcpy_async", "az_titan_offload"})
 
diff --git a/aozora_sdxl_training_amd/unet.py b/aozora_sdxl_training_amd/unet.py
--- a/aozora_sdxl_training_amd/unet.py
+++ b/aozora_sdxl_training_amd/unet.py
@@ -20,6 +20,7 @@
     side_batch: int = 1
     ln_fused: bool = True
     ln_defer: bool = True
+    ln_slabs: bool = True
     hoist: bool = True
     xkv_side: bool = True
     temb_side: bool = True
@@ -40,7 +41,7 @@
 
 
 class Act:
-    __slots__ = ("t", "g", "need_grad", "ready", "g_alias")
+    __slots__ = ("t", "g", "need_grad", "ready", "g_alias", "slab_ok", "slabs")
 
     def __init__(self, t: torch.Tensor, need_grad: bool = True):
         self.t = t
@@ -48,6 +49,8 @@
         self.need_grad = need_grad
         self.ready = None
         self.g_alias = False
+        self.slab_ok = False
+        self.slabs = None
 
 
 class _Pool:
@@ -517,6 +520,8 @@
             a.g = self._pool.get(tuple(a.t.shape), BF16)
             a.g_alias = False
             return a.g, None
+        if a.slabs is not None:
+            raise AozoraError("a second gradient contribution to an activation whose gradient lives in split-K slabs")
         if a.g_alias:
             old = a.g
             a.g = self._pool.get(tuple(a.t.shape), BF16)
@@ -674,8 +679,18 @@
             elif w_train or b_train:
                 self._side_defer(wgrad)
             if x.need_grad:
+                plan = (0, 0)
+                if self.policy.ln_slabs and x.slab_ok and x.g is None and not on_side and rows > 512:
+                    plan = ops.gemm_nt_split_plan(rows, WT.shape[0], WT.shape[1], dy.device)
                 dx, add = self._gbuf(x)
                 oop = add is not None and add is not dx
+                if plan[0] >= 2:
+                    if ops._ws_slot[0] != 0:
+                        raise AozoraError("slab data gradient issued outside the chain's workspace slot")
+                    x.slabs = (ops.gemm_nt_slabs(dy, WT, plan[0], plan[1]), lib().ncalls)
+                    if residual is not None:
+                        self._give_grad(residual, dy)
+                    return
 
                 def dgrad():
                     ops.gemm(dy, WT, dx, trans_b=True, accumulate=add is dx, residual=add if oop else None,
@@ -796,6 +811,8 @@
         stats = self._pool.get((2 * rows,), F32)
         gam, bet = self._w[prefix + ".weight"], self._w[prefix + ".bias"]
         ops.layernorm_fwd(x.t, gam, bet, y.t, stats, 1e-5)
+        y.slab_ok = (self.policy.ln_fused and self.policy.ln_defer and
+                     (self._trainable(prefix + ".weight") or self._trainable(prefix + ".bias")))
 
         def bwd():
             dy = y.g
@@ -805,6 +822,16 @@
             gw = self._gw[prefix + ".weight"] if self._trainable(prefix + ".weight") else None
             gb = self._gw[prefix + ".bias"] if self._trainable(prefix + ".bias") else None
             self._wait_ready(y)
+            if y.slabs is not None:
+                slabs, mark = y.slabs
+                y.slabs = None
+                nblk = ops.ln_partial_blocks(rows)
+                part = self._pool.get((nblk * C * 2,), F32)
+                if lib().ncalls != mark or ops._ws_slot[0] != 0:
+                    raise AozoraError("a launch came between a slab product and the LayerNorm backward that sums its slabs")
+                ops.layernorm_bwd_partial_slabs(x.t, gam, stats, slabs, dx, part, dx_add=add, nblk=nblk)
+                self._ln_jobs.append((part, gw, gb, nblk, C))
+                return
             if self.policy.ln_fused:
                 if self.policy.ln_defer:
                     nblk = ops.ln_partial_blocks(rows)
diff --git a/include/aozora_hip.h b/include/aozora_hip.h
--- a/include/aozora_hip.h
+++ b/include/aozora_hip.h
@@ -38,6 +38,10 @@
                  void* C, long ldc, const void* bias, const void* rowbias, int rows_per_seg, long ld_rowbias,
                  const void* residual, long ldr, int accumulate, int split_k, void* workspace, long workspace_bytes,
                  void* stream);
+
+int az_gemm_nt_split_plan(int M, int N, int K, long workspace_bytes, int* splits, int* bn);
+int az_gemm_nt_slabs_bf16(int M, int N, int K, const void* A, long lda, const void* B, long ldb, int splits, int bn,
+                          void* workspace, long workspace_bytes, void* stream);
 
 int az_gemm_nt_grouped_bf16(int M, int K, const void* A, long lda, const void* groups_dev, int ngroups, long total_tiles_n, void* stream);
 
@@ -86,6 +90,8 @@
                         void* stream);
 int az_layernorm_bwd_partial(int M, int C, const void* x, long ldx, const void* gamma, const void* stats, const void* dy,
                              long lddy, void* dx, long lddx, const void* dx_add, long ld_add, void* partial, int nblk, void* stream);
+int az_layernorm_bwd_partial_slabs(int M, int C, const void* x, long ldx, const void* gamma, const void* stats, const void* slabs, int splits,
+                                   void* dx, long lddx, const void* dx_add, long ld_add, void* partial, int nblk, void* stream);
 int az_ln_partial_blocks(int M);
 int az_ln_param_finish_multi(const void* jobs_dev, int njobs, long nblocks, void* stream);
 
```

Result: no change. 1.057 iters/sec (-0.1%).
